# ChainSafe/lumenos

Hardware: AMD Instinct MI355X
Metric: prove_eval_seconds_16384x4096 (lower is better)
Workload: dtype u64; 1 GPU; Encode+Commit+InnerProduct(r,b)+QueryCols 16384x4096 LogN=14 L=12 K=2 rhoInv=2 queries=309; parallelism=1 GPU: the whole job resident in HBM

## Files before the change

lumenos_amd/csrc/lm_common.h:

```cpp
#pragma once
#include <hip/hip_runtime.h>

#include <algorithm>
#include <cstdarg>
#include <cstdint>
#include <cstdio>
#include <map>
#include <memory>
#include <mutex>
#include <set>
#include <string>
#include <utility>
#include <vector>

#include "../../include/lumenos_hip.h"
#include "lm_arith.h"
#include "lm_dev.h"

#define LM_MAX_LIMBS LUMEN_MAX_LIMBS

struct lm_modmap {
    uint32_t period;
    uint8_t idx[LM_MAX_LIMBS];
};

struct lm_mods {
    mod_t m[LM_MAX_LIMBS];
};

struct lm_prof_entry {
    double total_ms = 0;
    uint64_t launches = 0;
    uint64_t units = 0;
};

struct lm_galois_key {
    lm_dev<u64> d_key;
    lm_dev<uint32_t> d_index;
    lm_dev<uint32_t> d_inv_index;
};

struct lumen_set {
    uint32_t count = 0;
    uint32_t nl = 0;
    uint32_t logw = 0;
    u64 *d = nullptr;
    size_t words = 0;
    bool owner = true;
    lumen_ctx *home = nullptr;
};

struct lm_shared {
    std::recursive_mutex mu;
    lm_dev<tw_t> tw_fwd;
    lm_dev<tw_t> tw_inv;
    std::vector<uint64_t> roots;
    uint32_t fieldN = 0;
    lm_dev<tw_t> scal;
    std::map<uint64_t, lm_galois_key> gkeys;
    std::map<std::string, std::shared_ptr<void>> ext;
};

struct lm_tuning {
    uint32_t ks_batch = 64;
    uint32_t ks_lanes = 0;
    int32_t ks_fused_digits = -1;
    uint32_t ks_close_fused = 1;
    uint32_t debug = 0;
    uint32_t modup_tgroup = 3, moddown_tgroup = 1;
    uint32_t ks_placement = 6;
    uint32_t batch_chunks = 0;
    uint32_t rccl_shared_device = 0;
};

struct lumen_ctx {
    lm_tuning tune;
    std::recursive_mutex mu;
    std::shared_ptr<lm_shared> sh;
    int device = 0;
    hipStream_t stream = nullptr;
    hipStream_t stream2 = nullptr;
    hipEvent_t ev_fork = nullptr, ev_join = nullptr;
    hipStream_t stream_aux = nullptr;
    hipEvent_t ev_aux = nullptr;
    hipEvent_t ev_xdep = nullptr;
    uint32_t aux_digests = 0;
    const u64 *aux_lo = nullptr, *aux_hi = nullptr;
    uint8_t *aux_host = nullptr;
    size_t aux_host_cap = 0;
    void *stage_host = nullptr;
    size_t stage_cap = 0;
    hipEvent_t ev_stage = nullptr;
    void *io_host[2] = {nullptr, nullptr};
    hipEvent_t ev_io[2] = {nullptr, nullptr};
    uint32_t logN = 0, N = 0, L = 0, K = 0;
    uint64_t T = 0;
    uint64_t mod[LM_MAX_LIMBS] = {0};
    uint64_t psi[LM_MAX_LIMBS] = {0};
    lm_mods mods;
    tw_t ninv[LM_MAX_LIMBS];
    std::vector<uint64_t> &roots;
    uint32_t &fieldN;
    std::map<uint64_t, lm_galois_key> &gkeys;
    std::map<std::string, std::shared_ptr<void>> &ext;
    uint64_t mul_counter = 0;
    std::map<std::string, lm_dev<unsigned char>> scratch;
    struct pool_block {
        void *p;
        hipEvent_t ready;
    };
    std::multimap<size_t, pool_block> pool;
    size_t pool_bytes = 0;
    std::set<const void *> lds_attr_done;
    bool prof = false;
    std::map<std::string, lm_prof_entry> prof_tab;
    struct pending_ev {
        std::string name;
        hipEvent_t a, b;
        uint64_t units;
    };
    std::vector<pending_ev> prof_pending;
    std::vector<hipEvent_t> ev_pool;
    hipEvent_t tm0 = nullptr, tm1 = nullptr;
    std::string err;
    explicit lumen_ctx(std::shared_ptr<lm_shared> s)
        : sh(std::move(s)), roots(sh->roots), fieldN(sh->fieldN), gkeys(sh->gkeys), ext(sh->ext) {}
};

static inline size_t lm_ctw(const lumen_ctx *ctx, const lumen_set *s);
#define LM_FULL_WIDTH(ctx, set, what) \
    LM_CHECK(ctx, (set)->logw == 0, "%s: lane-sharded set (1/%u of every limb) where a full-width set is required", what, 1u << (set)->logw)

#define LM_ENTER(ctx)                                             \
    std::lock_guard<std::recursive_mutex> lm_lock_((ctx)->mu);    \
    (void)hipSetDevice((ctx)->device);                            \
    (void)hipGetLastError()
#define LM_SHARED_LOCK(ctx) std::lock_guard<std::recursive_mutex> lm_shlock_((ctx)->sh->mu)

template <class T>
static inline std::shared_ptr<T> lm_ext_get(lumen_ctx *ctx, const std::string &key) {
    LM_SHARED_LOCK(ctx);
    auto it = ctx->ext.find(key);
    return it == ctx->ext.end() ? std::shared_ptr<T>() : std::static_pointer_cast<T>(it->second);
}
static inline void lm_ext_put(lumen_ctx *ctx, const std::string &key, std::shared_ptr<void> v) {
    LM_SHARED_LOCK(ctx);
    ctx->ext[key] = std::move(v);
}

static inline size_t lm_ctw(const lumen_ctx *ctx, const lumen_set *s) { return (size_t)2 * s->nl * (ctx->N >> s->logw); }

void lm_sync_all(lumen_ctx *ctx);
void *lm_stage(lumen_ctx *ctx, size_t bytes);
int lm_h2d_staged(lumen_ctx *ctx, void *dev, const void *host, size_t bytes);
bool lm_host_is_pinned(const void *p);
int lm_h2d(lumen_ctx *ctx, void *dev, const void *host, size_t bytes);
int lm_d2h(lumen_ctx *ctx, void *host, const void *dev, size_t bytes, bool wait);
int lm_h2d_rows(lumen_ctx *ctx, void *dev, size_t dpitch, const void *host, size_t spitch, size_t width, size_t height);

int lm_fail(lumen_ctx *ctx, const char *fmt, ...);
extern thread_local std::string lm_global_err;

#define LM_HIP(ctx, call)                                                                  \
    do {                                                                                   \
        hipError_t e_ = (call);                                                            \
        if (e_ != hipSuccess)                                                              \
            return lm_fail(ctx, "%s failed: %s (%s:%d)", #call, hipGetErrorString(e_),     \
                           __FILE__, __LINE__);                                            \
    } while (0)

#define LM_CHECK(ctx, cond, ...)                    \
    do {                                            \
        if (!(cond)) return lm_fail(ctx, __VA_ARGS__); \
    } while (0)

template <class... P, class... A>
static inline int lm_launch_flat(lumen_ctx *ctx, void (*kernel)(P...), size_t threads, A &&...args) {
    hipLaunchKernelGGL(kernel, dim3((uint32_t)((threads + 255) / 256)), dim3(256), 0, ctx->stream, std::forward<A>(args)...);
    LM_HIP(ctx, hipGetLastError());
    return 0;
}

struct lm_set_guard {
    lumen_ctx *ctx;
    lumen_set *s;
    lm_set_guard(lumen_ctx *c, lumen_set *x) : ctx(c), s(x) {}
    ~lm_set_guard() {
        if (s) lumen_set_destroy(ctx, s);
    }
    lumen_set *release() {
        lumen_set *r = s;
        s = nullptr;
        return r;
    }
    lm_set_guard(lm_set_guard &&o) : ctx(o.ctx), s(o.release()) {}
    lm_set_guard &operator=(const lm_set_guard &) = delete;
};

void lm_set_release_async(lumen_ctx *ctx, lumen_set *set);

void *lm_scratch(lumen_ctx *ctx, const char *name, size_t bytes);
void lm_scratch_adopt(lumen_ctx *ctx, const char *name, void *p, size_t bytes);

struct lm_prof_scope {
    lumen_ctx *ctx;
    const char *name;
    uint64_t units;
    hipEvent_t a = nullptr;
    lm_prof_scope(lumen_ctx *c, const char *n, uint64_t u);
    ~lm_prof_scope();
};
void lm_prof_resolve(lumen_ctx *ctx);

static inline uint64_t h_mulmod(uint64_t a, uint64_t b, uint64_t q) {
    return (uint64_t)(((u128)a * b) % q);
}
static inline uint64_t h_powmod(uint64_t a, uint64_t e, uint64_t q) {
    uint64_t r = 1 % q;
    a %= q;
    while (e) {
        if (e & 1) r = h_mulmod(r, a, q);
        a = h_mulmod(a, a, q);
        e >>= 1;
    }
    return r;
}
static inline uint64_t h_invmod(uint64_t a, uint64_t q) { return h_powmod(a, q - 2, q); }
static inline tw_t h_tw(uint64_t w, uint64_t q) {
    tw_t t;
    t.w = w;
    t.wp = (u64)((((u128)w) << 64) / q);
    return t;
}
static inline uint64_t h_r64_mod(uint64_t q) { return (uint64_t)((((u128)1) << 64) % q); }
static inline uint64_t h_p_mod(const lumen_ctx *ctx, uint64_t q) {
    uint64_t P = 1 % q;
    for (uint32_t a = 0; a < ctx->K; a++) P = h_mulmod(P, ctx->mod[ctx->L + a] % q, q);
    return P;
}
static inline uint32_t h_bitrev(uint32_t x, int bits) {
    uint32_t r = 0;
    for (int i = 0; i < bits; i++) r = (r << 1) | ((x >> i) & 1);
    return r;
}

int lm_launch_ntt(lumen_ctx *ctx, u64 *d, uint32_t npoly, const lm_modmap &map, bool inverse);
struct lm_ninv_t;
int lm_launch_ntt_strided(lumen_ctx *ctx, const u64 *src, size_t src_poly_stride, u64 *dst,
                          size_t dst_poly_stride, uint32_t npoly, const lm_modmap &map, bool inverse,
                          const char *prof_name, const lm_ninv_t *inv_scale = nullptr);
int lm_launch_ntt_subring(lumen_ctx *ctx, uint32_t logn, const tw_t *tw, tw_t ninv_scale, const u64 *src,
                          size_t src_poly_stride, u64 *dst, size_t dst_poly_stride, uint32_t npoly,
                          uint32_t mod_idx, bool inverse, const mod_t *explicit_mod = nullptr);
mod_t lm_make_mod(uint64_t q);
void lm_build_tw(uint64_t q, uint64_t psi, uint32_t logN, std::vector<tw_t> &fwd, std::vector<tw_t> &inv);
int lm_rescale_polys(lumen_ctx *ctx, const u64 *src, uint32_t nl, u64 *dst, uint32_t target,
                     uint32_t npoly, u64 *work, u64 *tbuf);
int lm_rescale_coef_ready(lumen_ctx *ctx);
int lm_rescale_polys_from_coef(lumen_ctx *ctx, const u64 *coef, uint32_t nl, u64 *dst, uint32_t target, uint32_t npoly);
lm_modmap lm_map_q(uint32_t nl);
lm_modmap lm_map_p(const lumen_ctx *ctx);
int lm_encode_dev(lumen_ctx *ctx, const lumen_set *matrix, const u64 *dzero, uint32_t rho_inv, lumen_set **encoded);
int lm_poly_eval_check(lumen_ctx *ctx, const uint64_t *values, uint32_t rows, uint32_t count, uint64_t first_column,
                       uint32_t cols, const char *what);
int lm_poly_eval_enqueue(lumen_ctx *ctx, const uint64_t *values, uint32_t rows, uint32_t count, uint64_t first_column,
                         uint32_t cols, uint64_t z, const char *what);
int lm_poly_eval_finish(lumen_ctx *ctx, uint64_t *partial);
hipEvent_t lm_ev_get(lumen_ctx *ctx);
```

lumenos_amd/csrc/lm_ctx.hip:

```cpp
#include <cstring>
#include <thread>

#include "lm_ntt_plan.h"

thread_local std::string lm_global_err;

int lm_fail(lumen_ctx *ctx, const char *fmt, ...) {
    char buf[1024];
    va_list ap;
    va_start(ap, fmt);
    vsnprintf(buf, sizeof(buf), fmt, ap);
    va_end(ap);
    if (ctx) ctx->err = buf;
    lm_global_err = buf;
    fprintf(stderr, "[lumenos_hip] error: %s\n", buf);
    return 1;
}

void *lm_scratch(lumen_ctx *ctx, const char *name, size_t bytes) {
    auto &e = ctx->scratch[name];
    if (e && e.count() >= bytes) return e.get();
    if (e) lm_sync_all(ctx);
    return e.alloc(ctx, bytes, name) ? nullptr : e.get();
}

void lm_scratch_adopt(lumen_ctx *ctx, const char *name, void *p, size_t bytes) {
    auto &e = ctx->scratch[name];
    if (e.get() == p) (void)e.release();
    if (e) lm_sync_all(ctx);
    e = lm_dev<unsigned char>((unsigned char *)p, bytes);
}

void lm_sync_all(lumen_ctx *ctx) {
    if (ctx->stream) hipStreamSynchronize(ctx->stream);
    if (ctx->stream2) hipStreamSynchronize(ctx->stream2);
    if (ctx->stream_aux) hipStreamSynchronize(ctx->stream_aux);
}

void *lm_stage(lumen_ctx *ctx, size_t bytes) {
    if (ctx->ev_stage) hipEventSynchronize(ctx->ev_stage);
    if (ctx->stage_cap < bytes) {
        if (ctx->stage_host) hipHostFree(ctx->stage_host);
        ctx->stage_host = nullptr, ctx->stage_cap = 0;
        if (hipHostMalloc(&ctx->stage_host, bytes, hipHostMallocDefault) != hipSuccess) {
            lm_fail(ctx, "hipHostMalloc(%zu) for host staging failed", bytes);
            return nullptr;
        }
        ctx->stage_cap = bytes;
    }
    return ctx->stage_host;
}

int lm_h2d_staged(lumen_ctx *ctx, void *dev, const void *host, size_t bytes) {
    void *h = lm_stage(ctx, bytes);
    if (!h) return 1;
    memcpy(h, host, bytes);
    LM_HIP(ctx, hipMemcpyAsync(dev, h, bytes, hipMemcpyHostToDevice, ctx->stream));
    LM_HIP(ctx, hipEventRecord(ctx->ev_stage, ctx->stream));
    return 0;
}

hipEvent_t lm_ev_get(lumen_ctx *ctx) {
    if (!ctx->ev_pool.empty()) {
        hipEvent_t e = ctx->ev_pool.back();
        ctx->ev_pool.pop_back();
        return e;
    }
    hipEvent_t e = nullptr;
    hipEventCreate(&e);
    return e;
}

lm_prof_scope::lm_prof_scope(lumen_ctx *c, const char *n, uint64_t u) : ctx(c), name(n), units(u) {
    if (!ctx->prof) return;
    a = lm_ev_get(ctx);
    hipEventRecord(a, ctx->stream);
}
lm_prof_scope::~lm_prof_scope() {
    if (!ctx->prof || !a) return;
    hipEvent_t b = lm_ev_get(ctx);
    hipEventRecord(b, ctx->stream);
    ctx->prof_pending.push_back({name, a, b, units});
}

void lm_prof_resolve(lumen_ctx *ctx) {
    if (ctx->prof_pending.empty()) return;
    for (auto &p : ctx->prof_pending) {
        float ms = 0;
        if (hipEventSynchronize(p.b) == hipSuccess && hipEventElapsedTime(&ms, p.a, p.b) == hipSuccess) {
            auto &e = ctx->prof_tab[p.name];
            e.total_ms += ms;
            e.launches += 1;
            e.units += p.units;
        } else {
            (void)hipGetLastError();
        }
        ctx->ev_pool.push_back(p.a);
        ctx->ev_pool.push_back(p.b);
    }
    ctx->prof_pending.clear();
}

lm_modmap lm_map_q(uint32_t nl) {
    lm_modmap m;
    m.period = nl;
    for (uint32_t i = 0; i < LM_MAX_LIMBS; i++) m.idx[i] = (uint8_t)(i < nl ? i : 0);
    return m;
}

lm_modmap lm_map_p(const lumen_ctx *ctx) {
    lm_modmap m;
    m.period = ctx->K;
    for (uint32_t i = 0; i < LM_MAX_LIMBS; i++) m.idx[i] = (uint8_t)(ctx->L + (i < ctx->K ? i : 0));
    return m;
}

mod_t lm_make_mod(uint64_t q) {
    mod_t m;
    m.q = q;
    m.qinv64 = (u64)((((u128)1) << 64) / q);
    u64 inv = 1;
    for (int it = 0; it < 6; it++) inv *= 2 - (u64)q * inv;
    m.qneg = (u64)0 - inv;
    u64 r = h_r64_mod(q);
    m.r2 = h_mulmod(r, r, q);
    return m;
}

void lm_build_tw(uint64_t q, uint64_t psi, uint32_t logN, std::vector<tw_t> &fwd, std::vector<tw_t> &inv) {
    uint32_t N = 1u << logN;
    fwd.resize(N);
    inv.resize(N);
    uint64_t psi_inv = h_invmod(psi, q), cf = 1, cb = 1;
    for (uint32_t j = 0; j < N; j++) {
        uint32_t r = h_bitrev(j, (int)logN);
        fwd[r] = h_tw(cf, q);
        inv[r] = h_tw(cb, q);
        cf = h_mulmod(cf, psi, q);
        cb = h_mulmod(cb, psi_inv, q);
    }
}

static void pool_drain(lumen_ctx *ctx) {
    for (auto &kv : ctx->pool) {
        hipFree(kv.second.p);
        if (kv.second.ready) ctx->ev_pool.push_back(kv.second.ready);
    }
    ctx->pool.clear();
    ctx->pool_bytes = 0;
}

static int ctx_private_init(lumen_ctx *ctx) {
    LM_HIP(ctx, hipSetDevice(ctx->device));
    LM_HIP(ctx, hipStreamCreate(&ctx->stream));
    LM_HIP(ctx, hipStreamCreate(&ctx->stream2));
    LM_HIP(ctx, hipEventCreateWithFlags(&ctx->ev_fork, hipEventDisableTiming));
    LM_HIP(ctx, hipEventCreateWithFlags(&ctx->ev_join, hipEventDisableTiming));
    LM_HIP(ctx, hipStreamCreate(&ctx->stream_aux));
    LM_HIP(ctx, hipEventCreateWithFlags(&ctx->ev_aux, hipEventDisableTiming));
    LM_HIP(ctx, hipEventCreateWithFlags(&ctx->ev_stage, hipEventDisableTiming));
    LM_HIP(ctx, hipEventCreateWithFlags(&ctx->ev_xdep, hipEventDisableTiming));
    LM_HIP(ctx, hipEventCreate(&ctx->tm0));
    LM_HIP(ctx, hipEventCreate(&ctx->tm1));
    return 0;
}

static int tuning_set(lm_tuning &t, const char *name, long v) {
    const std::string n(name ? name : "");
    auto in = [&](long lo, long hi) { return v >= lo && v <= hi; };
    if (n == "LUMEN_KS_BATCH") {
        if (!in(1, 4096)) return 2;
        t.ks_batch = (uint32_t)v;
    } else if (n == "LUMEN_KS_LANES") {
        if (!in(0, 2)) return 2;
        t.ks_lanes = (uint32_t)v;
    } else if (n == "LUMEN_KS_FUSED_DIGITS") {
        if (v > LM_MAX_LIMBS) return 2;
        t.ks_fused_digits = v >= 0 ? (int32_t)v : -1;
    } else if (n == "LUMEN_KS_CLOSE_FUSED") {
        if (!in(0, 1)) return 2;
        t.ks_close_fused = (uint32_t)v;
    } else if (n == "LUMEN_DEBUG") {
        t.debug = v != 0;
    } else if (n == "LUMEN_MODUP_TGROUP") {
        if (!in(1, 31)) return 2;
        t.modup_tgroup = (uint32_t)v;
    } else if (n == "LUMEN_MODDOWN_TGROUP") {
        if (!in(1, 31)) return 2;
        t.moddown_tgroup = (uint32_t)v;
    } else if (n == "LUMEN_KS_PLACEMENT") {
        if (!in(0, 32)) return 2;
        t.ks_placement = (uint32_t)v;
    } else if (n == "LUMEN_BATCH_CHUNKS") {
        if (!in(0, 4096)) return 2;
        t.batch_chunks = (uint32_t)v;
    } else {
        return 1;
    }
    return 0;
}
static void tuning_from_env(lm_tuning &t) {
    for (const char *n : {"LUMEN_KS_BATCH", "LUMEN_KS_LANES", "LUMEN_KS_FUSED_DIGITS", "LUMEN_KS_CLOSE_FUSED", "LUMEN_DEBUG",
                          "LUMEN_MODUP_TGROUP", "LUMEN_MODDOWN_TGROUP", "LUMEN_KS_PLACEMENT", "LUMEN_BATCH_CHUNKS"}) {
        const char *e = getenv(n);
        if (e && *e && tuning_set(t, n, atol(e)))
            fprintf(stderr, "[lumenos_hip] %s=%s is out of range: ignored\n", n, e);
    }
}

extern "C" int lumen_ctx_set_tuning(lumen_ctx *ctx, const char *name, long value) {
    LM_CHECK(nullptr, ctx && name, "lumen_ctx_set_tuning: NULL argument");
    LM_ENTER(ctx);
    const int rc = tuning_set(ctx->tune, name, value);
    LM_CHECK(ctx, rc != 1, "unknown tuning switch %s", name);
    LM_CHECK(ctx, rc == 0, "tuning switch %s: value %ld is out of range (nothing changed)", name, value);
    return 0;
}

extern "C" int lumen_test_allow_shared_device_rccl(lumen_ctx *ctx, int on) {
    LM_CHECK(nullptr, ctx, "lumen_test_allow_shared_device_rccl: NULL ctx");
    LM_ENTER(ctx);
    ctx->tune.rccl_shared_device = on != 0;
    return 0;
}

extern "C" int lumen_ctx_wait(lumen_ctx *ctx, lumen_ctx *other) {
    LM_CHECK(nullptr, ctx && other, "lumen_ctx_wait: NULL argument");
    if (ctx == other) return 0;
    hipEvent_t ev;
    {
        LM_ENTER(other);
        LM_HIP(other, hipEventRecord(other->ev_xdep, other->stream));
        ev = other->ev_xdep;
    }
    LM_ENTER(ctx);
    LM_CHECK(ctx, ctx->device == other->device, "lumen_ctx_wait: contexts on devices %d and %d", ctx->device, other->device);
    LM_HIP(ctx, hipStreamWaitEvent(ctx->stream, ev, 0));
    return 0;
}

extern "C" int lumen_ctx_create(const lumen_params_desc *desc, lumen_ctx **out) {
    if (!desc || !out) return lm_fail(nullptr, "lumen_ctx_create: NULL argument");
    *out = nullptr;
    LM_CHECK(nullptr, desc->abi_version == LUMEN_ABI_VERSION, "ABI version mismatch: got %u want %u",
             desc->abi_version, LUMEN_ABI_VERSION);
    LM_CHECK(nullptr, lm_logn_supported(desc->log_n) || lm_logn_split_supported(desc->log_n),
             "log_n %u unsupported: kernels are instantiated for N = 2^8 and 2^10..2^14, and the server's path and the key "
             "switch for N = 2^15",
             desc->log_n);
    LM_CHECK(nullptr, desc->num_q >= 1 && desc->num_q + desc->num_p <= LM_MAX_LIMBS,
             "bad limb counts L=%u K=%u", desc->num_q, desc->num_p);
    int ndev = 0;
    if (hipGetDeviceCount(&ndev) != hipSuccess || ndev == 0)
        return lm_fail(nullptr, "no HIP device visible: the lumenos HIP path has no CPU fallback");
    LM_CHECK(nullptr, desc->device >= 0 && desc->device < ndev, "device %d out of range (have %d)",
             desc->device, ndev);
    std::unique_ptr<lumen_ctx, void (*)(lumen_ctx *)> guard(new lumen_ctx(std::make_shared<lm_shared>()),
                                                            lumen_ctx_destroy);
    lumen_ctx *ctx = guard.get();
    tuning_from_env(ctx->tune);
    ctx->device = desc->device;
    ctx->logN = desc->log_n;
    ctx->N = 1u << desc->log_n;
    ctx->L = desc->num_q;
    ctx->K = desc->num_p;
    ctx->T = desc->plaintext_modulus;
    uint32_t LK = ctx->L + ctx->K, N = ctx->N;
    uint64_t two_n = 2ull * N;
    for (uint32_t i = 0; i < LK; i++) {
        uint64_t q = desc->moduli[i], psi = desc->psi[i];
        const uint64_t qmax = UINT64_MAX / lm_q_bound_factor(desc->log_n);
        if (q < (1ull << 20) || q > qmax || (q & (two_n - 1)) != 1)
            return lm_fail(nullptr, "modulus %u (%llu) must be == 1 mod 2N and below %llu", i,
                           (unsigned long long)q, (unsigned long long)qmax);
        if (h_powmod(psi, N, q) != q - 1)
            return lm_fail(nullptr, "psi[%u] is not a primitive 2N-th root of unity", i);
        ctx->mod[i] = q;
        ctx->psi[i] = psi;
        ctx->mods.m[i] = lm_make_mod(q);
        ctx->ninv[i] = h_tw(h_invmod(N % q, q), q);
    }
    for (uint32_t i = LK; i < LM_MAX_LIMBS; i++) ctx->mods.m[i] = ctx->mods.m[0];
    if (int rc = ctx_private_init(ctx)) return rc;
    std::vector<tw_t> f, b, fwd, inv;
    for (uint32_t i = 0; i < LK; i++) {
        lm_build_tw(ctx->mod[i], ctx->psi[i], ctx->logN, f, b);
        fwd.insert(fwd.end(), f.begin(), f.end());
        inv.insert(inv.end(), b.begin(), b.end());
    }
    lm_layout_tw(fwd, ctx->logN);
    lm_layout_tw(inv, ctx->logN);
    if (ctx->sh->tw_fwd.upload(ctx, fwd, "the forward twiddles") || ctx->sh->tw_inv.upload(ctx, inv, "the inverse twiddles")) return 1;
    *out = guard.release();
    return 0;
}

extern "C" int lumen_ctx_clone(lumen_ctx *src, lumen_ctx **out) {
    if (!src || !out) return lm_fail(nullptr, "lumen_ctx_clone: NULL argument");
    *out = nullptr;
    LM_ENTER(src);
    std::unique_ptr<lumen_ctx, void (*)(lumen_ctx *)> guard(new lumen_ctx(src->sh), lumen_ctx_destroy);
    lumen_ctx *ctx = guard.get();
    ctx->tune = src->tune;
    ctx->device = src->device;
    ctx->logN = src->logN, ctx->N = src->N, ctx->L = src->L, ctx->K = src->K, ctx->T = src->T;
    memcpy(ctx->mod, src->mod, sizeof(ctx->mod));
    memcpy(ctx->psi, src->psi, sizeof(ctx->psi));
    ctx->mods = src->mods;
    memcpy(ctx->ninv, src->ninv, sizeof(ctx->ninv));
    if (int rc = ctx_private_init(ctx)) {
        src->err = ctx->err;
        return rc;
    }
    *out = guard.release();
    return 0;
}

extern "C" void lumen_ctx_destroy(lumen_ctx *ctx) {
    if (!ctx) return;
    {
        LM_ENTER(ctx);
        lm_sync_all(ctx);
        ctx->scratch.clear();
        pool_drain(ctx);
        lm_prof_resolve(ctx);
        for (hipEvent_t e : ctx->ev_pool) hipEventDestroy(e);
        if (ctx->tm0) hipEventDestroy(ctx->tm0);
        if (ctx->tm1) hipEventDestroy(ctx->tm1);
        if (ctx->aux_host) hipHostFree(ctx->aux_host);
        if (ctx->stage_host) hipHostFree(ctx->stage_host);
        for (int i = 0; i < 2; i++) {
            if (ctx->io_host[i]) hipHostFree(ctx->io_host[i]);
            if (ctx->ev_io[i]) hipEventDestroy(ctx->ev_io[i]);
        }
        if (ctx->ev_stage) hipEventDestroy(ctx->ev_stage);
        if (ctx->ev_xdep) hipEventDestroy(ctx->ev_xdep);
        if (ctx->ev_aux) hipEventDestroy(ctx->ev_aux);
        if (ctx->stream_aux) hipStreamDestroy(ctx->stream_aux);
        if (ctx->ev_fork) hipEventDestroy(ctx->ev_fork);
        if (ctx->ev_join) hipEventDestroy(ctx->ev_join);
        if (ctx->stream2) hipStreamDestroy(ctx->stream2);
        if (ctx->stream) hipStreamDestroy(ctx->stream);
        ctx->sh.reset();
    }
    delete ctx;
}

extern "C" int lumen_ctx_trim(lumen_ctx *ctx) {
    LM_CHECK(nullptr, ctx, "lumen_ctx_trim: NULL ctx");
    LM_ENTER(ctx);
    LM_CHECK(ctx, !ctx->aux_digests, "lumen_ctx_trim: a lumen_leaf_digests_begin job is in flight");
    lm_sync_all(ctx);
    for (auto it = ctx->scratch.begin(); it != ctx->scratch.end();) {
        if (it->first == "digests_async" || it->first == "group_digests") {
            ++it;
            continue;
        }
        it = ctx->scratch.erase(it);
    }
    pool_drain(ctx);
    return 0;
}

extern "C" int lumen_ctx_scratch_info(lumen_ctx *ctx, const char *name, void **ptr, size_t *bytes) {
    LM_CHECK(nullptr, ctx && name && ptr, "lumen_ctx_scratch_info: NULL argument");
    LM_ENTER(ctx);
    auto it = ctx->scratch.find(name);
    *ptr = it == ctx->scratch.end() ? nullptr : it->second.get();
    if (bytes) *bytes = it == ctx->scratch.end() ? 0 : it->second.count();
    return 0;
}

extern "C" const char *lumen_last_error(const lumen_ctx *ctx) {
    return ctx ? ctx->err.c_str() : lm_global_err.c_str();
}

extern "C" int lumen_sync(lumen_ctx *ctx) {
    LM_CHECK(nullptr, ctx, "lumen_sync: NULL ctx");
    LM_ENTER(ctx);
    LM_HIP(ctx, hipStreamSynchronize(ctx->stream));
    return 0;
}

extern "C" uint64_t lumen_mul_counter(const lumen_ctx *ctx) { return ctx ? ctx->mul_counter : 0; }

extern "C" int lumen_set_create(lumen_ctx *ctx, uint32_t count, uint32_t num_limbs, lumen_set **out) {
    return lumen_set_create_lanes(ctx, count, num_limbs, 0, out);
}

extern "C" int lumen_set_create_lanes(lumen_ctx *ctx, uint32_t count, uint32_t num_limbs, uint32_t log_world,
                                      lumen_set **out) {
    LM_CHECK(nullptr, ctx && out, "lumen_set_create: NULL argument");
    LM_ENTER(ctx);
    LM_CHECK(ctx, num_limbs >= 1 && num_limbs <= ctx->L, "num_limbs %u out of range [1,%u]", num_limbs, ctx->L);
    LM_CHECK(ctx, log_world <= 6 && (ctx->N >> log_world) >= 64, "a lane shard of 1/%u of N = %u is narrower than 64 coefficients",
             1u << log_world, ctx->N);
    lumen_set *s = new lumen_set();
    s->count = count;
    s->nl = num_limbs;
    s->logw = log_world;
    s->words = (size_t)count * 2 * num_limbs * (ctx->N >> log_world);
    s->home = ctx;
    if (s->words) {
        const size_t bytes = s->words * sizeof(u64);
        auto it = ctx->pool.find(bytes);
        if (it != ctx->pool.end()) {
            s->d = (u64 *)it->second.p;
            if (hipEvent_t ready = it->second.ready) {
                (void)hipStreamWaitEvent(ctx->stream, ready, 0);
                (void)hipStreamWaitEvent(ctx->stream2, ready, 0);
                (void)hipStreamWaitEvent(ctx->stream_aux, ready, 0);
                ctx->ev_pool.push_back(ready);
            }
            ctx->pool.erase(it);
            ctx->pool_bytes -= bytes;
        } else {
            hipError_t e = hipMalloc((void **)&s->d, bytes);
            if (e != hipSuccess && !ctx->pool.empty()) {
                (void)hipGetLastError();
                lm_sync_all(ctx);
                pool_drain(ctx);
                e = hipMalloc((void **)&s->d, bytes);
            }
            if (e != hipSuccess) {
                (void)hipGetLastError();
                delete s;
                return lm_fail(ctx, "hipMalloc(%zu bytes) for a %u x %u-limb set failed: %s", bytes, count,
                               num_limbs, hipGetErrorString(e));
            }
        }
    }
    *out = s;
    return 0;
}

extern "C" void lumen_set_destroy(lumen_ctx *ctx, lumen_set *set) {
    if (!set) return;
    if (ctx) {
        LM_ENTER(ctx);
        hipStreamSynchronize(ctx->stream);
        hipStreamSynchronize(ctx->stream2);
        if (ctx->aux_digests && set->d && set->d < ctx->aux_hi && set->d + set->words > ctx->aux_lo)
            hipStreamSynchronize(ctx->stream_aux);
        if (set->owner && set->d) {
            const size_t bytes = set->words * sizeof(u64);
            if (ctx == set->home && ctx->pool_bytes + bytes <= ((size_t)96 << 30)) {
                ctx->pool.emplace(bytes, lumen_ctx::pool_block{set->d, nullptr});
                ctx->pool_bytes += bytes;
            } else {
                hipFree(set->d);
            }
        }
    } else if (set->owner && set->d) {
        hipFree(set->d);
    }
    delete set;
}

void lm_set_release_async(lumen_ctx *ctx, lumen_set *set) {
    if (!set) return;
    LM_ENTER(ctx);
    const size_t bytes = set->words * sizeof(u64);
    const bool hashing = ctx->aux_digests && set->d && set->d < ctx->aux_hi && set->d + set->words > ctx->aux_lo;
    if (!set->owner || !set->d || ctx != set->home || hashing || ctx->pool_bytes + bytes > ((size_t)96 << 30)) {
        lumen_set_destroy(ctx, set);
        return;
    }
    hipEvent_t ready = lm_ev_get(ctx);
    bool ok = ready && hipEventRecord(ctx->ev_join, ctx->stream2) == hipSuccess &&
              hipStreamWaitEvent(ctx->stream, ctx->ev_join, 0) == hipSuccess && hipEventRecord(ready, ctx->stream) == hipSuccess;
    if (!ok) {
        (void)hipGetLastError();
        if (ready) ctx->ev_pool.push_back(ready);
        lumen_set_destroy(ctx, set);
        return;
    }
    ctx->pool.emplace(bytes, lumen_ctx::pool_block{set->d, ready});
    ctx->pool_bytes += bytes;
    delete set;
}

extern "C" int lumen_set_slice(lumen_ctx *ctx, const lumen_set *set, uint32_t first, uint32_t n,
                               lumen_set **view) {
    LM_CHECK(nullptr, ctx && set && view, "lumen_set_slice: NULL argument");
    LM_ENTER(ctx);
    LM_CHECK(ctx, (uint64_t)first + n <= set->count, "slice [%u,%u) exceeds set of %u", first, first + n, set->count);
    lumen_set *v = new lumen_set();
    const size_t ctw = lm_ctw(ctx, set);
    v->count = n;
    v->nl = set->nl;
    v->logw = set->logw;
    v->d = set->d + (size_t)first * ctw;
    v->words = (size_t)n * ctw;
    v->owner = false;
    *view = v;
    return 0;
}

extern "C" uint32_t lumen_set_count(const lumen_set *set) { return set ? set->count : 0; }
extern "C" uint32_t lumen_set_limbs(const lumen_set *set) { return set ? set->nl : 0; }
extern "C" uint32_t lumen_set_log_world(const lumen_set *set) { return set ? set->logw : 0; }
extern "C" void *lumen_set_device_ptr(const lumen_set *set) { return set ? set->d : nullptr; }

extern "C" void *lumen_host_alloc(size_t bytes) {
    void *p = nullptr;
    if (hipHostMalloc(&p, bytes ? bytes : 1, hipHostMallocDefault) != hipSuccess) {
        (void)hipGetLastError();
        lm_fail(nullptr, "hipHostMalloc(%zu) failed", bytes);
        return nullptr;
    }
    return p;
}
extern "C" void lumen_host_free(void *p) {
    if (p) hipHostFree(p);
}

static int host_limbs_move(uint64_t *flat, uint64_t *const *limbs, size_t n, size_t words, uint32_t threads, bool gather) {
    if (!n || !words) return 0;
    const size_t bytes = words * sizeof(uint64_t);
    size_t nthr = threads ? threads : std::max(1u, std::min(16u, std::thread::hardware_concurrency()));
    nthr = std::min(nthr, n);
    auto work = [=](size_t lo, size_t hi) {
        for (size_t i = lo; i < hi; i++) {
            if (gather) memcpy(flat + i * words, limbs[i], bytes);
            else memcpy(limbs[i], flat + i * words, bytes);
        }
    };
    if (nthr == 1) {
        work(0, n);
        return 0;
    }
    std::vector<std::thread> th;
    for (size_t t = 0; t < nthr; t++) th.emplace_back(work, n * t / nthr, n * (t + 1) / nthr);
    for (auto &x : th) x.join();
    return 0;
}
extern "C" int lumen_host_gather(uint64_t *dst, const uint64_t *const *limbs, size_t n, size_t words, uint32_t threads) {
    LM_CHECK(nullptr, (dst && limbs) || !n, "lumen_host_gather: NULL argument");
    for (size_t i = 0; i < n; i++) LM_CHECK(nullptr, limbs[i], "lumen_host_gather: limb %zu is NULL", i);
    return host_limbs_move(dst, const_cast<uint64_t *const *>(limbs), n, words, threads, true);
}
extern "C" int lumen_host_scatter(const uint64_t *src, uint64_t *const *limbs, size_t n, size_t words, uint32_t threads) {
    LM_CHECK(nullptr, (src && limbs) || !n, "lumen_host_scatter: NULL argument");
    for (size_t i = 0; i < n; i++) LM_CHECK(nullptr, limbs[i], "lumen_host_scatter: limb %zu is NULL", i);
    return host_limbs_move(const_cast<uint64_t *>(src), limbs, n, words, threads, false);
}

bool lm_host_is_pinned(const void *p) {
    hipPointerAttribute_t a;
    if (hipPointerGetAttributes(&a, p) != hipSuccess) {
        (void)hipGetLastError();
        return false;
    }
    return a.type == hipMemoryTypeHost;
}

#define LM_IO_CHUNK ((size_t)64 << 20)
static void par_memcpy(void *dst, const void *src, size_t bytes) {
    const size_t nthr = bytes >= ((size_t)8 << 20) ? 4 : 1;
    if (nthr == 1) {
        memcpy(dst, src, bytes);
        return;
    }
    std::thread th[4];
    const size_t part = (bytes / nthr + 63) & ~(size_t)63;
    for (size_t t = 0; t < nthr; t++) {
        const size_t lo = std::min(bytes, t * part), hi = std::min(bytes, lo + part);
        th[t] = std::thread([=] { memcpy((char *)dst + lo, (const char *)src + lo, hi - lo); });
    }
    for (size_t t = 0; t < nthr; t++) th[t].join();
}

static int io_buffers(lumen_ctx *ctx) {
    for (int i = 0; i < 2; i++) {
        if (!ctx->io_host[i]) LM_HIP(ctx, hipHostMalloc(&ctx->io_host[i], LM_IO_CHUNK, hipHostMallocDefault));
        if (!ctx->ev_io[i]) LM_HIP(ctx, hipEventCreateWithFlags(&ctx->ev_io[i], hipEventDisableTiming));
    }
    return 0;
}

int lm_h2d(lumen_ctx *ctx, void *dev, const void *host, size_t bytes) {
    char *dst = (char *)dev;
    if (bytes <= ((size_t)1 << 20) || lm_host_is_pinned(host)) {
        LM_HIP(ctx, hipMemcpyAsync(dst, host, bytes, hipMemcpyHostToDevice, ctx->stream));
    } else {
        if (int rc = io_buffers(ctx)) return rc;
        int i = 0;
        for (size_t off = 0; off < bytes; off += LM_IO_CHUNK, i ^= 1) {
            const size_t len = std::min(LM_IO_CHUNK, bytes - off);
            LM_HIP(ctx, hipEventSynchronize(ctx->ev_io[i]));
            par_memcpy(ctx->io_host[i], (const char *)host + off, len);
            LM_HIP(ctx, hipMemcpyAsync(dst + off, ctx->io_host[i], len, hipMemcpyHostToDevice, ctx->stream));
            LM_HIP(ctx, hipEventRecord(ctx->ev_io[i], ctx->stream));
        }
    }
    LM_HIP(ctx, hipStreamSynchronize(ctx->stream));
    return 0;
}

int lm_h2d_rows(lumen_ctx *ctx, void *dev, size_t dpitch, const void *host, size_t spitch, size_t width, size_t height) {
    char *dst = (char *)dev;
    const char *src = (const char *)host;
    if (!width || !height) return 0;
    if (width * height <= ((size_t)1 << 20) || lm_host_is_pinned(host)) {
        LM_HIP(ctx, hipMemcpy2DAsync(dst, dpitch, src, spitch, width, height, hipMemcpyHostToDevice, ctx->stream));
    } else {
        LM_CHECK(ctx, width <= LM_IO_CHUNK, "lm_h2d_rows: a row of %zu bytes exceeds the bounce buffer", width);
        if (int rc = io_buffers(ctx)) return rc;
        const size_t per = LM_IO_CHUNK / width;
        int i = 0;
        for (size_t r = 0; r < height; r += per, i ^= 1) {
            const size_t nr = std::min(per, height - r);
            LM_HIP(ctx, hipEventSynchronize(ctx->ev_io[i]));
            if (spitch == width)
                par_memcpy(ctx->io_host[i], src + r * spitch, nr * width);
            else
                for (size_t k = 0; k < nr; k++) memcpy((char *)ctx->io_host[i] + k * width, src + (r + k) * spitch, width);
            LM_HIP(ctx, hipMemcpy2DAsync(dst + r * dpitch, dpitch, ctx->io_host[i], width, width, nr, hipMemcpyHostToDevice,
                                         ctx->stream));
            LM_HIP(ctx, hipEventRecord(ctx->ev_io[i], ctx->stream));
        }
    }
    LM_HIP(ctx, hipStreamSynchronize(ctx->stream));
    return 0;
}

extern "C" int lumen_set_upload(lumen_ctx *ctx, lumen_set *set, uint32_t first, uint32_t n,
                                const uint64_t *host) {
    LM_CHECK(nullptr, ctx && set && host, "lumen_set_upload: NULL argument");
    LM_ENTER(ctx);
    LM_CHECK(ctx, (uint64_t)first + n <= set->count, "upload range [%u,%u) exceeds set of %u", first, first + n, set->count);
    const size_t ctw = lm_ctw(ctx, set), bytes = (size_t)n * ctw * sizeof(u64);
    return lm_h2d(ctx, set->d + (size_t)first * ctw, host, bytes);
}

int lm_d2h(lumen_ctx *ctx, void *host, const void *dev, size_t bytes, bool wait) {
    const char *src = (const char *)dev;
    if (bytes <= ((size_t)1 << 20) || lm_host_is_pinned(host)) {
        LM_HIP(ctx, hipMemcpyAsync(host, src, bytes, hipMemcpyDeviceToHost, ctx->stream));
        if (wait || !lm_host_is_pinned(host)) LM_HIP(ctx, hipStreamSynchronize(ctx->stream));
        return 0;
    }
    if (int rc = io_buffers(ctx)) return rc;
    const size_t nchunks = (bytes + LM_IO_CHUNK - 1) / LM_IO_CHUNK;
    auto issue = [&](size_t k) -> int {
        const size_t off = k * LM_IO_CHUNK, len = std::min(LM_IO_CHUNK, bytes - off);
        LM_HIP(ctx, hipMemcpyAsync(ctx->io_host[k & 1], src + off, len, hipMemcpyDeviceToHost, ctx->stream));
        LM_HIP(ctx, hipEventRecord(ctx->ev_io[k & 1], ctx->stream));
        return 0;
    };
    if (nchunks)
        if (int rc = issue(0)) return rc;
    for (size_t k = 0; k < nchunks; k++) {
        if (k + 1 < nchunks)
            if (int rc = issue(k + 1)) return rc;
        const size_t off = k * LM_IO_CHUNK, len = std::min(LM_IO_CHUNK, bytes - off);
        LM_HIP(ctx, hipEventSynchronize(ctx->ev_io[k & 1]));
        par_memcpy((char *)host + off, ctx->io_host[k & 1], len);
    }
    return 0;
}

extern "C" int lumen_set_download(lumen_ctx *ctx, const lumen_set *set, uint32_t first, uint32_t n,
                                  uint64_t *host) {
    LM_CHECK(nullptr, ctx && set && host, "lumen_set_download: NULL argument");
    LM_ENTER(ctx);
    LM_CHECK(ctx, (uint64_t)first + n <= set->count, "download range [%u,%u) exceeds set of %u", first, first + n, set->count);
    const size_t ctw = lm_ctw(ctx, set), bytes = (size_t)n * ctw * sizeof(u64);
    return lm_d2h(ctx, host, set->d + (size_t)first * ctw, bytes, true);
}

__global__ void k_fill_random(u64 *d, size_t words, uint32_t N, uint32_t nl, lm_mods mods, u64 seed) {
    size_t i = (size_t)blockIdx.x * blockDim.x + threadIdx.x;
    size_t stride = (size_t)gridDim.x * blockDim.x;
    for (; i < words; i += stride) {
        uint32_t limb = (uint32_t)((i / N) % nl);
        u64 z = seed + 0x9e3779b97f4a7c15ull * (u64)(i + 1);
        z = (z ^ (z >> 30)) * 0xbf58476d1ce4e5b9ull;
        z = (z ^ (z >> 27)) * 0x94d049bb133111ebull;
        z ^= z >> 31;
        d[i] = lm_reduce(z, mods.m[limb].q, mods.m[limb].qinv64);
    }
}

extern "C" int lumen_set_fill_random(lumen_ctx *ctx, lumen_set *set, uint64_t seed) {
    LM_CHECK(nullptr, ctx && set, "lumen_set_fill_random: NULL argument");
    LM_ENTER(ctx);
    if (!set->words) return 0;
    hipLaunchKernelGGL(k_fill_random, dim3(2048), dim3(256), 0, ctx->stream, set->d, set->words,
                       ctx->N >> set->logw, set->nl, ctx->mods, (u64)seed);
    LM_HIP(ctx, hipGetLastError());
    return 0;
}

extern "C" int lumen_timer_start(lumen_ctx *ctx) {
    LM_CHECK(nullptr, ctx, "NULL ctx");
    LM_ENTER(ctx);
    LM_HIP(ctx, hipEventRecord(ctx->tm0, ctx->stream));
    return 0;
}

extern "C" int lumen_timer_stop(lumen_ctx *ctx, float *elapsed_ms) {
    LM_CHECK(nullptr, ctx && elapsed_ms, "NULL argument");
    LM_ENTER(ctx);
    LM_HIP(ctx, hipEventRecord(ctx->tm1, ctx->stream));
    LM_HIP(ctx, hipEventSynchronize(ctx->tm1));
    LM_HIP(ctx, hipEventElapsedTime(elapsed_ms, ctx->tm0, ctx->tm1));
    return 0;
}

extern "C" int lumen_prof_enable(lumen_ctx *ctx, int on) {
    LM_CHECK(nullptr, ctx, "NULL ctx");
    LM_ENTER(ctx);
    if (!on) lm_prof_resolve(ctx);
    ctx->prof = on != 0;
    return 0;
}

extern "C" int lumen_prof_reset(lumen_ctx *ctx) {
    LM_CHECK(nullptr, ctx, "NULL ctx");
    LM_ENTER(ctx);
    lm_prof_resolve(ctx);
    ctx->prof_tab.clear();
    return 0;
}

extern "C" size_t lumen_prof_names(lumen_ctx *ctx, char *buf, size_t cap) {
    if (!ctx) return 0;
    LM_ENTER(ctx);
    lm_prof_resolve(ctx);
    std::string all;
    for (auto &kv : ctx->prof_tab) {
        if (!all.empty()) all += ",";
        all += kv.first;
    }
    if (buf && cap) {
        size_t n = std::min(cap - 1, all.size());
        memcpy(buf, all.data(), n);
        buf[n] = 0;
    }
    return all.size();
}

extern "C" int lumen_prof_read(lumen_ctx *ctx, const char *kernel, double *total_ms,
                               uint64_t *launches, uint64_t *units) {
    LM_CHECK(nullptr, ctx && kernel, "NULL argument");
    LM_ENTER(ctx);
    lm_prof_resolve(ctx);
    auto it = ctx->prof_tab.find(kernel);
    lm_prof_entry e;
    if (it != ctx->prof_tab.end()) e = it->second;
    if (total_ms) *total_ms = e.total_ms;
    if (launches) *launches = e.launches;
    if (units) *units = e.units;
    return 0;
}
```

lumenos_amd/csrc/lm_innersum.hip:

```cpp
#include <algorithm>

#include "lm_ks_host.h"

__global__ __launch_bounds__(256) void k_acc_canon(u64 *__restrict__ acc, size_t pairs, uint32_t logN, uint32_t L, lm_mods mods) {
    const size_t stride = (size_t)gridDim.x * blockDim.x;
    for (size_t g = (size_t)blockIdx.x * blockDim.x + threadIdx.x; g < pairs; g += stride) {
        const u64 q = mods.m[(uint32_t)((g >> (logN - 1)) % L)].q;
        ulonglong2 v = *reinterpret_cast<ulonglong2 *>(acc + 2 * g);
        v.x = lm_csub(v.x, q), v.y = lm_csub(v.y, q);
        *reinterpret_cast<ulonglong2 *>(acc + 2 * g) = v;
    }
}

__global__ __launch_bounds__(256) void k_lazy_gather(const u64 *__restrict__ u, const u64 *__restrict__ cur, u64 *__restrict__ lazy,
                                                     const uint32_t *__restrict__ index, uint32_t B, uint32_t L, uint32_t K,
                                                     uint32_t pshift, uint32_t logN, uint32_t first, lm_mods mods) {
    const uint32_t N = 1u << logN, nq = L * 2 * B;
    const size_t total = (size_t)2 * B * (L + K) * (N / 2), stride = (size_t)gridDim.x * blockDim.x;
    for (size_t g = (size_t)blockIdx.x * blockDim.x + threadIdx.x; g < total; g += stride) {
        const uint32_t j = (uint32_t)(g & (N / 2 - 1)) * 2, limb = (uint32_t)(g >> (logN - 1));
        const uint32_t t = limb < nq ? limb / (2 * B) : L + (limb - nq) % K;
        const uint32_t pw = limb < nq ? limb % (2 * B) : (limb - nq) / K;
        const bool with_c = t < L && (pw & 1) == (u ? 0u : 1u);
        if (!u && !with_c) continue;
        const u64 q = mods.m[ks_mod_at(t, L, pshift)].q;
        const size_t o = ((size_t)limb << logN) + j;
        uint2 p;
        p.x = j, p.y = j + 1;
        if (index) p = *reinterpret_cast<const uint2 *>(index + j);
        ulonglong2 v;
        v.x = v.y = 0;
        if (!first) v = *reinterpret_cast<const ulonglong2 *>(lazy + o);
        if (u) v.x += u[((size_t)limb << logN) + p.x], v.y += u[((size_t)limb << logN) + p.y];
        if (with_c) {
            const u64 *c = cur + (((size_t)pw * L + t) << logN);
            v.x += c[p.x], v.y += c[p.y];
        }
        v.x = lm_csub(lm_csub(v.x, 2 * q), q), v.y = lm_csub(lm_csub(v.y, 2 * q), q);
        *reinterpret_cast<ulonglong2 *>(lazy + o) = v;
    }
}

namespace {

int acc_canon(lumen_ctx *ctx, u64 *acc, size_t words, uint32_t L) {
    if (!words) return 0;
    hipLaunchKernelGGL(k_acc_canon, dim3(2048), dim3(256), 0, ctx->stream, acc, words / 2, ctx->logN, L, ctx->mods);
    LM_HIP(ctx, hipGetLastError());
    return 0;
}


bool is_plain(const lumen_ctx *ctx, uint32_t batch, uint32_t n) { return batch == 1 && n && !(n & (n - 1)) && n <= ctx->N; }

template <class Fn>
int sum_walk(const lumen_ctx *ctx, uint32_t batch, uint32_t n, Fn &&fn) {
    if (is_plain(ctx, batch, n)) {
        uint64_t gal[64];
        const uint32_t cnt = lumen_inner_sum_galois_elements(ctx, n, gal);
        for (uint32_t r = 0; r < cnt; r++)
            if (int rc = fn((uint64_t)0, gal[r])) return rc;
        return 0;
    }
    for (uint32_t i = 0, j = n; j > 1; i++, j >>= 1) {
        const uint64_t term = (j & 1) ? lumen_galois_element(ctx, (int64_t)((uint64_t)(n - (n & ((2u << i) - 1))) * batch)) : 0;
        if (int rc = fn(term, lumen_galois_element(ctx, (int64_t)((uint64_t)batch << i)))) return rc;
    }
    return 0;
}

struct SumPlan {
    struct Step {
        const lm_galois_key *dbl = nullptr, *term = nullptr;
    } it[32];
    uint32_t cnt = 0;
    uint64_t last_el = 0;
    bool lazy = false;
};

int sum_plan(lumen_ctx *ctx, uint32_t batch, uint32_t n, SumPlan *p) {
    return sum_walk(ctx, batch, n, [&](uint64_t term, uint64_t dbl) {
        SumPlan::Step &st = p->it[p->cnt++];
        if (term) {
            if (int rc = ks_find_key(ctx, term, &st.term)) return rc;
            p->lazy = true;
        }
        p->last_el = dbl;
        return ks_find_key(ctx, dbl, &st.dbl);
    });
}

int general_check(lumen_ctx *ctx, uint32_t batch, uint32_t n, const char *what) {
    LM_CHECK(ctx, batch >= 1 && n >= 1, "%s: batch size %u and length %u must both be at least 1", what, batch, n);
    LM_CHECK(ctx, ctx->K >= 1, "parameters have no special primes: key switching unavailable");
    LM_CHECK(ctx, ctx->K <= 2, "key switching supports 1 or 2 special primes (have %u)", ctx->K);
    if (is_plain(ctx, batch, n)) return 0;
    LM_CHECK(ctx, (uint64_t)batch * n <= ctx->N / 2, "%s: batch size %u x length %u spans beyond the slot row of %u slots", what, batch, n,
             ctx->N / 2);
    return 0;
}


int lazy_blocks(lumen_ctx *ctx, const KsRun &run, u64 **lazy) {
    const size_t bytes = (size_t)run.Bmax * 2 * (ctx->L + ctx->K) * ctx->N * 8;
    lazy[0] = (u64 *)lm_scratch(ctx, "ks_lazy", bytes);
    lazy[1] = run.lanes > 1 ? (u64 *)lm_scratch(ctx, "ks_lazy_b", bytes) : lazy[0];
    return lazy[0] && lazy[1] ? 0 : 1;
}

int lazy_gather(lumen_ctx *ctx, const u64 *u, const u64 *cur, u64 *lazy, const uint32_t *index, bool first, uint32_t B, KsTables *tb) {
    lm_prof_scope ps(ctx, "ks_lazy_gather", (uint64_t)B);
    hipLaunchKernelGGL(k_lazy_gather, dim3(2048), dim3(256), 0, ctx->stream, u, cur, lazy, index, B, tb->nl, ctx->K, ctx->L - tb->nl,
                       ctx->logN, first ? 1u : 0u, ctx->mods);
    LM_HIP(ctx, hipGetLastError());
    return 0;
}

int identity_tables(lumen_ctx *ctx, std::shared_ptr<lm_galois_key> *out) {
    static const char *const NAME = "ks_identity";
    LM_SHARED_LOCK(ctx);
    auto gk = lm_ext_get<lm_galois_key>(ctx, NAME);
    if (!gk) {
        gk = std::make_shared<lm_galois_key>();
        std::vector<uint32_t> index(ctx->N);
        for (uint32_t i = 0; i < ctx->N; i++) index[i] = i;
        if (gk->d_index.upload(ctx, index, "the identity's index table") || gk->d_inv_index.upload(ctx, index, "the identity's index table"))
            return 1;
        lm_ext_put(ctx, NAME, gk);
    }
    *out = std::move(gk);
    return 0;
}

int lazy_close(lumen_ctx *ctx, const u64 *cur, u64 *out, u64 *lazy, uint32_t B, KsTables *tb, const KsScratch &s) {
    std::shared_ptr<lm_galois_key> id;
    if (int rc = identity_tables(ctx, &id)) return rc;
    if (int rc = lazy_gather(ctx, nullptr, cur, lazy, nullptr, false, B, tb)) return rc;
    if (int rc = rotate_p_to_coef(ctx, lazy, B, tb)) return rc;
    KsScratch sl = s;
    sl.u = lazy;
    return rotate_store(ctx, cur, out, B, *id, tb, sl);
}

int inner_sum_batch(lumen_ctx *ctx, u64 *acc, uint32_t B, const SumPlan &plan, KsTables *tb, const KsScratch &s, u64 *lazy,
                    u64 *close_out) {
    LM_CHECK(ctx, !close_out || (plan.cnt && !plan.lazy), "InnerSum has no rotation to close");
    u64 *cur = acc, *other = s.acc2;
    bool first = true;
    for (uint32_t r = 0; r < plan.cnt; r++) {
        const SumPlan::Step &st = plan.it[r];
        if (int rc = rotate_decompose(ctx, cur, B, tb, s)) return rc;
        if (st.term) {
            if (int rc = rotate_mac(ctx, cur, B, *st.term, tb, s)) return rc;
            if (int rc = lazy_gather(ctx, s.u, cur, lazy, st.term->d_index.get(), first, B, tb)) return rc;
            first = false;
        }
        if (close_out && r + 1 == plan.cnt)
            return rotate_close(ctx, cur, close_out, B, *st.dbl, plan.last_el, tb, s);
        if (int rc = rotate_add(ctx, cur, other, B, *st.dbl, tb, s)) return rc;
        std::swap(cur, other);
    }
    if (plan.lazy) {
        if (int rc = lazy_close(ctx, cur, other, lazy, B, tb, s)) return rc;
        std::swap(cur, other);
    }
    if (cur != acc)
        LM_HIP(ctx, hipMemcpyAsync(acc, cur, (size_t)B * 2 * tb->nl * ctx->N * 8, hipMemcpyDeviceToDevice, ctx->stream));
    return 0;
}

int check_inner_sum_level(lumen_ctx *ctx, const lumen_set *in, const char *what) {
    LM_FULL_WIDTH(ctx, in, what);
    LM_CHECK(ctx, in->nl == ctx->L, "%s is implemented at the top level only (set has %u of %u limbs)", what,
             in->nl, ctx->L);
    return 0;
}

int inner_sum_run(lumen_ctx *ctx, const lumen_set *in, uint32_t batch, uint32_t n, const char *general, lumen_set **out) {
    if (general) {
        if (int rc = general_check(ctx, batch, n, general)) return rc;
    } else {
        LM_CHECK(ctx, is_plain(ctx, batch, n), "InnerSum length %u is not a power of two <= N", n);
    }
    KsRun run;
    if (int rc = ks_run_open(ctx, in->count, in->nl, is_plain(ctx, batch, n) ? 1 : 2, false, &run)) return rc;
    SumPlan plan;
    if (in->count)
        if (int rc = sum_plan(ctx, batch, n, &plan)) return rc;
    lumen_set *o = nullptr;
    if (int rc = lumen_set_create(ctx, in->count, in->nl, &o)) return rc;
    lm_set_guard og(ctx, o);
    if (in->words)
        LM_HIP(ctx, hipMemcpyAsync(o->d, in->d, in->words * 8, hipMemcpyDeviceToDevice, ctx->stream));
    if (int rc = ks_run_scratch(ctx, &run)) return rc;
    u64 *lazy[2] = {nullptr, nullptr};
    if (plan.lazy)
        if (int rc = lazy_blocks(ctx, run, lazy)) return rc;
    const size_t ctw = (size_t)2 * in->nl * ctx->N;
    auto batch_fn = [&](uint32_t, uint32_t first, uint32_t B, const KsScratch &s, u64 *) {
        return inner_sum_batch(ctx, o->d + (size_t)first * ctw, B, plan, run.tb, s, lazy[&s == &run.s[1]], nullptr);
    };
    if (int rc = ks_run(ctx, run, in->count, ctw, batch_fn)) return rc;
    if (!plan.lazy)
        if (int rc = acc_canon(ctx, o->d, o->words, in->nl)) return rc;
    *out = og.release();
    return 0;
}

int matrix_inner_sum_run(lumen_ctx *ctx, const lumen_set *matrix, const uint64_t *pt, uint32_t rows, const char *general,
                         lumen_set **out) {
    if (general) {
        if (int rc = general_check(ctx, 1, rows, general)) return rc;
    } else {
        LM_CHECK(ctx, is_plain(ctx, 1, rows), "rows=%u is not a power of two <= N", rows);
    }
    KsRun run;
    if (int rc = ks_run_open(ctx, matrix->count, matrix->nl, 2, true, &run)) return rc;
    SumPlan plan;
    if (matrix->count)
        if (int rc = sum_plan(ctx, 1, rows, &plan)) return rc;
    u64 *ptT = nullptr;
    if (int rc = upload_ptT(ctx, pt, matrix->nl, &ptT)) return rc;
    const uint32_t N = ctx->N, L = matrix->nl, target = std::min<uint32_t>(2, L);
    lumen_set *o = nullptr;
    if (int rc = lumen_set_create(ctx, matrix->count, target, &o)) return rc;
    lm_set_guard og(ctx, o);
    const size_t ctw = (size_t)2 * L * N, octw = (size_t)2 * target * N;
    if (int rc = ks_run_scratch(ctx, &run)) return rc;
    u64 *lazy[2] = {nullptr, nullptr};
    if (plan.lazy)
        if (int rc = lazy_blocks(ctx, run, lazy)) return rc;
    u64 *work = (u64 *)lm_scratch(ctx, "rescale_work", run.group_bytes);
    u64 *tbuf = (u64 *)lm_scratch(ctx, "rescale_t", (size_t)run.group * 2 * N * 8);
    if (!work || !tbuf) return 1;
    bool close = false;
    if (L > target && rows > 1 && ctx->tune.ks_close_fused && !plan.lazy && !lm_is_split(ctx->logN)) {
        const int rc = lm_rescale_coef_ready(ctx);
        if (rc && rc != 2) return rc;
        close = rc == 0;
    }
    auto batch_fn = [&](uint32_t g0, uint32_t first, uint32_t B, const KsScratch &s, u64 *a) {
        if (int rc = launch_mul_plain(ctx, matrix->d + (size_t)(g0 + first) * ctw, a, ptT, (size_t)B * ctw, L, B))
            return rc;
        return inner_sum_batch(ctx, a, B, plan, run.tb, s, lazy[&s == &run.s[1]], close ? work + (size_t)first * ctw : nullptr);
    };
    auto end_of_group = [&](uint32_t g0, uint32_t gn) {
        if (close)
            return lm_rescale_polys_from_coef(ctx, work, L, o->d + (size_t)g0 * octw, target, gn * 2);
        if (L > target) return lm_rescale_polys(ctx, run.acc, L, o->d + (size_t)g0 * octw, target, gn * 2, work, tbuf);
        if (!plan.lazy)
            if (int rc = acc_canon(ctx, run.acc, (size_t)gn * ctw, L)) return rc;
        LM_HIP(ctx, hipMemcpyAsync(o->d + (size_t)g0 * octw, run.acc, (size_t)gn * ctw * 8, hipMemcpyDeviceToDevice, ctx->stream));
        return 0;
    };
    if (int rc = ks_run(ctx, run, matrix->count, ctw, batch_fn, end_of_group)) return rc;
    *out = og.release();
    return 0;
}

}

extern "C" int lumen_inner_sum_general(lumen_ctx *ctx, const lumen_set *in, uint32_t batch_size, uint32_t n, lumen_set **out) {
    LM_CHECK(nullptr, ctx && in && out, "lumen_inner_sum_general: NULL argument");
    LM_ENTER(ctx);
    if (int rc = check_level_of_chain(ctx, in, "InnerSum")) return rc;
    return inner_sum_run(ctx, in, batch_size, n, "lumen_inner_sum_general", out);
}

extern "C" int lumen_matrix_inner_sum_general(lumen_ctx *ctx, const lumen_set *matrix, const uint64_t *pt, uint32_t rows,
                                              lumen_set **out) {
    LM_CHECK(nullptr, ctx && matrix && pt && out, "lumen_matrix_inner_sum_general: NULL argument");
    LM_ENTER(ctx);
    if (int rc = check_level_of_chain(ctx, matrix, "matrixInnerSumEval")) return rc;
    return matrix_inner_sum_run(ctx, matrix, pt, rows, "lumen_matrix_inner_sum_general", out);
}

extern "C" uint32_t lumen_inner_sum_general_elements(const lumen_ctx *ctx, uint32_t batch_size, uint32_t n, uint64_t *gal_els) {
    if (!ctx || !gal_els) return 0;
    if (!is_plain(ctx, batch_size, n) && (!batch_size || !n || (uint64_t)batch_size * n > ctx->N / 2)) return 0;
    uint32_t cnt = 0;
    sum_walk(ctx, batch_size, n, [&](uint64_t term, uint64_t dbl) {
        for (uint64_t g : {term, dbl})
            if (g > 1 && std::find(gal_els, gal_els + cnt, g) == gal_els + cnt) gal_els[cnt++] = g;
        return 0;
    });
    return cnt;
}

extern "C" int lumen_inner_sum(lumen_ctx *ctx, const lumen_set *in, uint32_t n, lumen_set **out) {
    LM_CHECK(nullptr, ctx && in && out, "lumen_inner_sum: NULL argument");
    LM_ENTER(ctx);
    if (int rc = check_inner_sum_level(ctx, in, "InnerSum")) return rc;
    return inner_sum_run(ctx, in, 1, n, nullptr, out);
}

extern "C" int lumen_inner_sum_at_level(lumen_ctx *ctx, const lumen_set *in, uint32_t n, lumen_set **out) {
    LM_CHECK(nullptr, ctx && in && out, "lumen_inner_sum_at_level: NULL argument");
    LM_ENTER(ctx);
    if (int rc = check_level_of_chain(ctx, in, "InnerSum")) return rc;
    return inner_sum_run(ctx, in, 1, n, nullptr, out);
}

extern "C" int lumen_matrix_inner_sum(lumen_ctx *ctx, const lumen_set *matrix, const uint64_t *pt,
                                      uint32_t rows, lumen_set **out) {
    LM_CHECK(nullptr, ctx && matrix && pt && out, "lumen_matrix_inner_sum: NULL argument");
    LM_ENTER(ctx);
    if (int rc = check_inner_sum_level(ctx, matrix, "matrixInnerSumEval")) return rc;
    return matrix_inner_sum_run(ctx, matrix, pt, rows, nullptr, out);
}

extern "C" int lumen_matrix_inner_sum_at_level(lumen_ctx *ctx, const lumen_set *matrix, const uint64_t *pt,
                                               uint32_t rows, lumen_set **out) {
    LM_CHECK(nullptr, ctx && matrix && pt && out, "lumen_matrix_inner_sum_at_level: NULL argument");
    LM_ENTER(ctx);
    if (int rc = check_level_of_chain(ctx, matrix, "matrixInnerSumEval")) return rc;
    return matrix_inner_sum_run(ctx, matrix, pt, rows, nullptr, out);
}
```

lumenos_amd/csrc/lm_keyswitch.hip:

```cpp
#include <cstdlib>
#include <cstring>

#include "lm_ks_host.h"

__device__ __forceinline__ u32 bx_v(u128 A, u128 M, u64 y0, u64 y1, u64 m0, u64 m1) {
    const u128 D1 = A >= M ? A - M : M - A, D2 = 2 * M - A;
    if ((u64)(D1 >> 64) >= 8 && (u64)(D2 >> 64) >= 8) return A >= M ? 1u : 0u;
    double vf = 0.0;
    vf += (double)y0 / (double)m0;
    vf += (double)y1 / (double)m1;
    return (u32)(u64)vf;
}

__device__ __forceinline__ void pack_pair(u64 a, u64 b, u64 m0, u64 m1, u128 M, u64 &hi, u64 &lo) {
    u64 l1, h1, l2, h2;
    mul128(a, m1, l1, h1);
    mul128(b, m0, l2, h2);
    const u128 A = (((u128)h1 << 64) | l1) + (((u128)h2 << 64) | l2);
    const u32 v = bx_v(A, M, a, b, m0, m1);
    const u128 W = A + (v == 0 ? 2 * M : (v == 1 ? M : (u128)0));
    hi = (u64)(W >> LM_W_SPLIT), lo = (u64)W & ((1ull << LM_W_SPLIT) - 1);
}

__global__ __launch_bounds__(256) void k_pack_v(u64 *__restrict__ y, size_t poly_stride, uint32_t npoly,
                                                uint32_t ngroups, uint32_t group_limbs, uint32_t first_mod,
                                                uint32_t nlimbs_total, uint32_t logN, lm_mods mods) {
    const uint32_t N = 1u << logN;
    const size_t total = (size_t)npoly * ngroups * (N / 2), stride = (size_t)gridDim.x * blockDim.x;
    for (size_t g = (size_t)blockIdx.x * blockDim.x + threadIdx.x; g < total; g += stride) {
        const uint32_t i = (uint32_t)(g & (N / 2 - 1)) * 2;
        const uint32_t grp = (uint32_t)((g >> (logN - 1)) % ngroups), p = (uint32_t)((g >> (logN - 1)) / ngroups);
        const uint32_t l0 = grp * group_limbs;
        if (l0 + 1 >= nlimbs_total) continue;
        u64 *y0 = y + (size_t)p * poly_stride + (size_t)l0 * N + i;
        const ulonglong2 av = *reinterpret_cast<const ulonglong2 *>(y0);
        const ulonglong2 bv = *reinterpret_cast<const ulonglong2 *>(y0 + N);
        const u64 m0 = mods.m[first_mod + l0].q, m1 = mods.m[first_mod + l0 + 1].q;
        u64 Ml, Mh;
        mul128(m0, m1, Ml, Mh);
        const u128 M = ((u128)Mh << 64) | Ml;
        ulonglong2 hv, lv;
#pragma unroll
        for (int e = 0; e < 2; e++) {
            const u64 a = e ? av.y : av.x, b = e ? bv.y : bv.x;
            u64 hi, lo;
            pack_pair(a, b, m0, m1, M, hi, lo);
            if (e) hv.y = hi, lv.y = lo;
            else hv.x = hi, lv.x = lo;
        }
        *reinterpret_cast<ulonglong2 *>(y0) = hv;
        *reinterpret_cast<ulonglong2 *>(y0 + N) = lv;
    }
}

template <int LOGN>
__global__ LM_GEOM_BOUNDS(lm_geom_lds(LOGN)) void k_intt_pack(const u64 *__restrict__ acc, u64 *coef, uint32_t B,
                                                                  uint32_t L, uint32_t nf, lm_mods mods,
                                                                  lm_ninv_t yscale, const tw_t *__restrict__ tw_all) {
    extern __shared__ __attribute__((aligned(16))) u64 sm[];
    constexpr uint32_t N = 1u << LOGN;
    const uint32_t tid = threadIdx.x;
    if (blockIdx.x >= B * nf) {
        const uint32_t k = blockIdx.x - B * nf, l = 2 * nf + k / B, b = k % B;
        const u64 *p = acc + (((size_t)b * 2 + 1) * L + l) * N;
        u64 *o = coef + ((size_t)b * L + l) * N;
        const lm_qc q = lm_make_qc(mods.m[l]);
        const tw_t sc = yscale.t[l];
        auto ld = [&](uint32_t i0, u64 *v, int count) { lm_load_run(p, i0, v, count); };
        auto st = [&](uint32_t i, u64 v) { o[i] = lm_shoup_cs(v, sc, q.q, q.nq); };
        lm_ntt_inverse<LOGN>(sm, tw_all + (size_t)l * N, q, tid, ld, st);
        return;
    }
    const uint32_t d = blockIdx.x / B, b = blockIdx.x % B;
    const uint32_t l0 = 2 * d, l1 = l0 + 1;
    const u64 *c1 = acc + ((size_t)b * 2 + 1) * L * N;
    u64 *o0 = coef + ((size_t)b * L + l0) * N;
    const lm_qc q0 = lm_make_qc(mods.m[l0]);
    const tw_t s0 = yscale.t[l0];
    {
        const u64 *p = c1 + (size_t)l0 * N;
        auto ld = [&](uint32_t i0, u64 *v, int count) { lm_load_run(p, i0, v, count); };
        auto st = [&](uint32_t i, u64 v) { o0[i] = lm_shoup_cs(v, s0, q0.q, q0.nq); };
        lm_ntt_inverse<LOGN>(sm, tw_all + (size_t)l0 * N, q0, tid, ld, st);
    }
    __syncthreads();
    {
        const lm_qc q1 = lm_make_qc(mods.m[l1]);
        const tw_t s1 = yscale.t[l1];
        const u64 *p = c1 + (size_t)l1 * N;
        u64 Ml, Mh;
        mul128(q0.q, q1.q, Ml, Mh);
        auto uni = [](u64 x) {
            return (u64)(uint32_t)__builtin_amdgcn_readfirstlane((int)(uint32_t)x) |
                   (u64)(uint32_t)__builtin_amdgcn_readfirstlane((int)(uint32_t)(x >> 32)) << 32;
        };
        const u128 M = ((u128)uni(Mh) << 64) | uni(Ml);
        auto ld = [&](uint32_t i0, u64 *v, int count) { lm_load_run(p, i0, v, count); };
        constexpr int R_LAST = lm_pass_r(LOGN, 0), LOG_T0 = LOGN - R_LAST;
        constexpr int PF = (1 << R_LAST) * 5 / 8;
        struct pack_t {
            u64 *o0;
            const lm_qc &q0, &q1;
            tw_t s1;
            u128 M;
            u64 y0[PF];
            __device__ __forceinline__ void pre(uint32_t w) {
#pragma unroll
                for (int k = 0; k < PF; k++) y0[k] = o0[w + ((uint32_t)k << LOG_T0)];
            }
            __device__ __forceinline__ void operator()(uint32_t i, u64 v, int k) {
                const u64 y1 = lm_shoup_cs(v, s1, q1.q, q1.nq);
                uint32_t j = i;
                asm volatile("" : "+v"(j));
                const u64 a = k < PF ? y0[k < PF ? k : 0] : o0[j];
                u64 hi, lo;
                pack_pair(a, y1, q0.q, q1.q, M, hi, lo);
                o0[j] = hi, o0[j + N] = lo;
                if (k >= PF && (k & 1)) asm volatile("" ::: "memory");
            }
        } st{o0, q0, q1, s1, M, {}};
        uint32_t tid1 = tid;
        asm volatile("" : "+v"(tid1));
        lm_ntt_inverse<LOGN>(sm, tw_all + (size_t)l1 * N, q1, tid1, ld, st);
    }
}

template <int LOGN>
__global__ LM_GEOM_BOUNDS(lm_geom_fwd(LOGN)) void k_modup_ntt(const u64 *__restrict__ coef, const u64 *__restrict__ acc,
                                                    u64 *__restrict__ ext, const bx_t *__restrict__ bx,
                                                    uint32_t B, uint32_t L, uint32_t K, uint32_t beta, uint32_t pshift,
                                                    const uint32_t *__restrict__ work, lm_mods mods,
                                                    const tw_t *__restrict__ tw_all) {
    extern __shared__ __attribute__((aligned(16))) u64 sm[];
    constexpr uint32_t N = 1u << LOGN;
    const uint32_t tid = threadIdx.x, LK = L + K;
    const lm_half<LOGN> hf = lm_half_of_block<LOGN>();
    const uint32_t wk = work[hf.block];
    const uint32_t b = wk & 0xFFFF, d = (wk >> 16) & 0xFF, t = wk >> 24;
    const uint32_t mt = ks_mod_at(t, L, pshift);
    const bx_t c = bx[d * LK + t];
    u64 *o = ext + ks_ext_at(b, d, t, B, beta) * N + hf.off;
    const lm_qc qc = lm_make_qc(mods.m[mt]);
    const u64 *s0 = coef + ((size_t)b * L + d * K) * N;
    const u64 *s1 = c.ns == 2 ? s0 + N : s0;
    auto ld = [&](uint32_t i) { return bx_apply(c, s0[i], s1[i], qc); };
    auto out = [&](uint32_t j, u64 v0, u64 v1) {
        ulonglong2 y;
        y.x = v0, y.y = v1;
        *reinterpret_cast<ulonglong2 *>(o + j) = y;
    };
    if constexpr (LOGN == 14) {
        lm_w14_runs st{sm};
        auto after = [&](uint32_t i0, uint32_t) { lm_w14_linear_out(sm, tid, i0, out); };
        lm_ntt_forward_w14(sm, tw_all + (size_t)mt * N, qc, tid, ld, st, after);
    } else {
        lm_lds_runs st{sm};
        auto after = [&](uint32_t, uint32_t) { lm_linear_out<lm_tlog(LOGN)>(sm, tid, out); };
        lm_ntt_forward_half<LOGN>(sm, tw_all + (size_t)mt * N, qc, tid, hf, ld, st, after);
    }
}

#ifndef LM_MAC_COLS
#define LM_MAC_COLS 4
#endif
#ifndef LM_MAC_VEC
#define LM_MAC_VEC 1
#endif
#ifndef LM_MAC_PREFETCH
#define LM_MAC_PREFETCH 1
#endif
template <int VEC>
struct mac_vec;
template <>
struct mac_vec<1> {
    u64 v[1];
    static __device__ __forceinline__ mac_vec load(const u64 *p) { return mac_vec{{*p}}; }
    static __device__ __forceinline__ mac_vec load_once(const u64 *p) { return mac_vec{{__builtin_nontemporal_load(p)}}; }
    __device__ __forceinline__ void store(u64 *p) const { *p = v[0]; }
};
template <>
struct mac_vec<2> {
    u64 v[2];
    static __device__ __forceinline__ mac_vec load(const u64 *p) {
        const ulonglong2 a = *reinterpret_cast<const ulonglong2 *>(p);
        return mac_vec{{a.x, a.y}};
    }
    static __device__ __forceinline__ mac_vec load_once(const u64 *p) {
        return mac_vec{{__builtin_nontemporal_load(p), __builtin_nontemporal_load(p + 1)}};
    }
    __device__ __forceinline__ void store(u64 *p) const {
        ulonglong2 a;
        a.x = v[0], a.y = v[1];
        *reinterpret_cast<ulonglong2 *>(p) = a;
    }
};
struct mac_acc {
    u64 a0, a1, a3;
    u32 c0, c1;
    __device__ __forceinline__ void clear() { a0 = a1 = a3 = 0, c0 = c1 = 0; }
    __device__ __forceinline__ void value(u64 &lo, u64 &hi) const {
        lo = a0 + (a1 << 32);
        hi = a3 + c0 + (a1 >> 32) + ((u64)c1 << 32) + (lo < a0 ? 1 : 0);
    }
};
__device__ __forceinline__ void mac2(mac_acc &p, mac_acc &q, u64 x, u64 k0, u64 k1) {
    const u32 x0 = (u32)x, x1 = (u32)(x >> 32);
#if LM_ASM_SHOUP
    asm("v_mad_u64_u32 %[pa0], s[98:99], %[x0], %[k00], %[pa0]\n\t"
        "v_mad_u64_u32 %[qa0], s[90:91], %[x0], %[k10], %[qa0]\n\t"
        "v_mad_u64_u32 %[pa1], s[94:95], %[x0], %[k01], %[pa1]\n\t"
        "v_addc_co_u32_e64 %[pc0], s[96:97], %[pc0], 0, s[98:99]\n\t"
        "v_mad_u64_u32 %[qa1], s[92:93], %[x0], %[k11], %[qa1]\n\t"
        "v_addc_co_u32_e64 %[qc0], s[96:97], %[qc0], 0, s[90:91]\n\t"
        "v_mad_u64_u32 %[pa3], s[96:97], %[x1], %[k01], %[pa3]\n\t"
        "v_addc_co_u32_e64 %[pc1], s[96:97], %[pc1], 0, s[94:95]\n\t"
        "v_mad_u64_u32 %[pa1], s[98:99], %[x1], %[k00], %[pa1]\n\t"
        "v_addc_co_u32_e64 %[qc1], s[96:97], %[qc1], 0, s[92:93]\n\t"
        "v_mad_u64_u32 %[qa1], s[90:91], %[x1], %[k10], %[qa1]\n\t"
        "v_mad_u64_u32 %[qa3], s[96:97], %[x1], %[k11], %[qa3]\n\t"
        "v_addc_co_u32_e64 %[pc1], s[96:97], %[pc1], 0, s[98:99]\n\t"
        "v_addc_co_u32_e64 %[qc1], s[96:97], %[qc1], 0, s[90:91]"
        : [pa0] "+v"(p.a0), [pa1] "+v"(p.a1), [pa3] "+v"(p.a3), [pc0] "+v"(p.c0), [pc1] "+v"(p.c1),
          [qa0] "+v"(q.a0), [qa1] "+v"(q.a1), [qa3] "+v"(q.a3), [qc0] "+v"(q.c0), [qc1] "+v"(q.c1)
        : [x0] "v"(x0), [x1] "v"(x1), [k00] "v"((u32)k0), [k01] "v"((u32)(k0 >> 32)), [k10] "v"((u32)k1),
          [k11] "v"((u32)(k1 >> 32))
        : "s92", "s93", "s94", "s95", "s96", "s97", "s98", "s99", "s90", "s91");
#else
    auto one = [&](mac_acc &r, u64 k) {
        const u32 k0w = (u32)k, k1w = (u32)(k >> 32);
        u64 t = r.a0 + (u64)x0 * k0w;
        r.c0 += t < r.a0, r.a0 = t;
        t = r.a1 + (u64)x0 * k1w;
        r.c1 += t < r.a1, r.a1 = t;
        t = r.a1 + (u64)x1 * k0w;
        r.c1 += t < r.a1, r.a1 = t;
        r.a3 += (u64)x1 * k1w;
    };
    one(p, k0);
    one(q, k1);
#endif
}

__global__ __launch_bounds__(256) void k_ks_mac(const u64 *__restrict__ ext, const u64 *__restrict__ acc,
                                                const u64 *__restrict__ key, u64 *__restrict__ u, uint32_t B,
                                                uint32_t L, uint32_t K, uint32_t beta, uint32_t pshift,
                                                uint32_t key_beta, uint32_t logN, lm_mods mods) {
    typedef mac_vec<LM_MAC_VEC> vec;
    const uint32_t N = 1u << logN, LK = L + K;
    const uint32_t G = (B + LM_MAC_COLS - 1) / LM_MAC_COLS, per_limb = N / (256 * LM_MAC_VEC) ? N / (256 * LM_MAC_VEC) : 1;
    const uint32_t slices = per_limb * LK;
    uint32_t slice, z;
    if (slices % 8 == 0) {
        const uint32_t xcd = blockIdx.x & 7, j = blockIdx.x >> 3;
        z = j % G;
        slice = (j / G) * 8 + xcd;
    } else {
        z = blockIdx.x % G;
        slice = blockIdx.x / G;
    }
    const uint32_t i = ((slice % per_limb) * 256 + threadIdx.x) * LM_MAC_VEC;
    const uint32_t t = LK - 1 - slice / per_limb;
    const uint32_t mt = ks_mod_at(t, L, pshift);
    const uint32_t b0 = z * LM_MAC_COLS;
    if (i >= N) return;
    const mod_t md = mods.m[mt];
    const uint32_t own = t < L ? t / K : 0xFFFFFFFFu;
    mac_acc a0[LM_MAC_COLS][LM_MAC_VEC], a1[LM_MAC_COLS][LM_MAC_VEC];
#pragma unroll
    for (int c = 0; c < LM_MAC_COLS; c++)
#pragma unroll
        for (int e = 0; e < LM_MAC_VEC; e++) a0[c][e].clear(), a1[c][e].clear();
    struct digit_t {
        vec k0, k1, x[LM_MAC_COLS];
    };
    auto fetch = [&](uint32_t d) {
        digit_t g;
        g.k0 = vec::load(key + ks_key_at(d, 0, mt, key_beta) * N + i);
        g.k1 = vec::load(key + ks_key_at(d, 1, mt, key_beta) * N + i);
#pragma unroll
        for (int c = 0; c < LM_MAC_COLS; c++) {
            const uint32_t bc = b0 + c < B ? b0 + c : B - 1;
            g.x[c] = d == own ? vec::load(acc + ((size_t)(bc * 2 + 1) * L + t) * N + i)
                              : vec::load_once(ext + ks_ext_at(bc, d, t, B, beta) * N + i);
        }
        return g;
    };
    constexpr int PF = LM_MAC_PREFETCH;
    digit_t q[PF + 1];
#pragma unroll
    for (int j = 0; j < PF; j++)
        if ((uint32_t)j < beta) q[j] = fetch(j);
    for (uint32_t d0 = 0; d0 < beta; d0 += PF + 1) {
#pragma unroll
        for (int j = 0; j <= PF; j++) {
            const uint32_t d = d0 + j;
            if (d < beta) {
                if (d + PF < beta) q[(j + PF) % (PF + 1)] = fetch(d + PF);
#pragma unroll
                for (int c = 0; c < LM_MAC_COLS; c++)
#pragma unroll
                    for (int e = 0; e < LM_MAC_VEC; e++) mac2(a0[c][e], a1[c][e], q[j].x[c].v[e], q[j].k0.v[e], q[j].k1.v[e]);
            }
        }
    }
#pragma unroll
    for (int c = 0; c < LM_MAC_COLS; c++) {
        if (b0 + c < B) {
            u64 *o = u + ks_u_at((b0 + c) * 2, t, B, L, K) * N + i, *o1 = u + ks_u_at((b0 + c) * 2 + 1, t, B, L, K) * N + i;
            vec r0, r1;
#pragma unroll
            for (int e = 0; e < LM_MAC_VEC; e++) {
                u64 lo, hi;
                a0[c][e].value(lo, hi);
                r0.v[e] = lm_mont_reduce_wide(lo, hi, md.q, md.qneg, md.qinv64, beta);
                a1[c][e].value(lo, hi);
                r1.v[e] = lm_mont_reduce_wide(lo, hi, md.q, md.qneg, md.qinv64, beta);
            }
            r0.store(o);
            r1.store(o1);
        }
    }
}

template <int LOGN, bool ACCUMULATE>
__device__ __forceinline__ void moddown_body(const u64 *__restrict__ u, const u64 *__restrict__ acc_in,
                                             u64 *__restrict__ acc_out, const bx_t *__restrict__ bxp,
                                             const tw_t *__restrict__ pinv,
                                             const uint32_t *__restrict__ index,
                                             const uint32_t *__restrict__ inv_index,
                                             const uint32_t *__restrict__ work, uint32_t B,
                                             uint32_t L, uint32_t K, const lm_mods &mods,
                                             const tw_t *__restrict__ tw_all) {
    extern __shared__ __attribute__((aligned(16))) u64 sm[];
    constexpr uint32_t N = 1u << LOGN;
    const uint32_t tid = threadIdx.x;
    const lm_half<LOGN> hf = lm_half_of_block<LOGN>();
    const uint32_t wk = work[hf.block];
    const uint32_t pw = wk & 0xFFFF;
    const uint32_t t = wk >> 16;
    const uint32_t w = pw & 1;
    const bx_t c = bxp[t];
    const lm_qc qc = lm_make_qc(mods.m[t]);
    const u64 *up0 = u + ks_u_at(pw, L, B, L, K) * N;
    const u64 *up1 = c.ns == 2 ? up0 + N : up0;
    const u64 *uq = u + ks_u_at(pw, t, B, L, K) * N;
    const u64 *ain = acc_in + ((size_t)pw * L + t) * N;
    u64 *aout = acc_out + ((size_t)pw * L + t) * N;
    tw_t pi = pinv[t];
    pi.w = qc.q - pi.w, pi.wp = ~pi.wp;
    auto ld = [&](uint32_t i) { return bx_apply(c, up0[i], up1[i], qc); };
    if constexpr (LOGN == 14) {
        const uint32_t wave = tid >> 6, lane = tid & 63;
        const uint32_t jb0 = (uint32_t)__builtin_amdgcn_readfirstlane((int)(inv_index[(2 * wave) << 10] >> 10));
        const uint32_t jb1 = (uint32_t)__builtin_amdgcn_readfirstlane((int)(inv_index[(2 * wave + 1) << 10] >> 10));
        lm_w14_runs st{sm};
        auto after = [&](uint32_t i0h, uint32_t) {
            const uint32_t pb = LM_PAD((wave << 10) | (2 * lane));
            constexpr uint32_t CH = 4;
            const uint32_t i = (wave << 11) | i0h | (2 * lane);
            const uint32_t jb = i0h ? jb1 : jb0, sbase = wave << 10;
#pragma unroll
            for (uint32_t k0 = 0; k0 < 8; k0 += CH) {
                ulonglong2 uv[CH], cv[CH];
#pragma unroll
                for (uint32_t k = 0; k < CH; k++) {
                    uv[k] = *reinterpret_cast<const ulonglong2 *>(uq + i + 128 * (k0 + k));
                    if (w == 0) cv[k] = *reinterpret_cast<const ulonglong2 *>(ain + i + 128 * (k0 + k));
                }
#pragma unroll
                for (uint32_t k = 0; k < CH; k++) {
                    const uint32_t p = lm_w14_at(pb, 128 * (k0 + k));
                    const u64 a0 = w == 0 ? uv[k].x + cv[k].x : uv[k].x, a1 = w == 0 ? uv[k].y + cv[k].y : uv[k].y;
                    sm[p] = lm_shoup3<true>(sm[p], pi.w, pi.wp, qc.nq, a0);
                    sm[p + 1] = lm_shoup3<true>(sm[p + 1], pi.w, pi.wp, qc.nq, a1);
                }
                LM_W14_FENCE();
            }
            lm_wave_sync();
            uint2 p[8];
            ulonglong2 x[8];
#pragma unroll
            for (uint32_t k = 0; k < 8; k++) {
                const uint32_t j = (jb << 10) + 2 * lane + k * 128;
                p[k] = *reinterpret_cast<const uint2 *>(index + j);
                if constexpr (ACCUMULATE) x[k] = *reinterpret_cast<const ulonglong2 *>(ain + j);
            }
#pragma unroll
            for (uint32_t k = 0; k < 8; k++) {
                const uint32_t j = (jb << 10) + 2 * lane + k * 128;
                ulonglong2 y;
                if constexpr (ACCUMULATE) {
                    y.x = lm_csub(lm_csub(x[k].x + sm[LM_PAD(sbase | (p[k].x & 1023u))], 4 * qc.q), 2 * qc.q);
                    y.y = lm_csub(lm_csub(x[k].y + sm[LM_PAD(sbase | (p[k].y & 1023u))], 4 * qc.q), 2 * qc.q);
                } else {
                    y.x = lm_csub(lm_csub(lm_csub(sm[LM_PAD(sbase | (p[k].x & 1023u))], 4 * qc.q), 2 * qc.q), qc.q);
                    y.y = lm_csub(lm_csub(lm_csub(sm[LM_PAD(sbase | (p[k].y & 1023u))], 4 * qc.q), 2 * qc.q), qc.q);
                }
                *reinterpret_cast<ulonglong2 *>(aout + j) = y;
            }
        };
        lm_ntt_forward_w14(sm, tw_all + (size_t)t * N, qc, tid, ld, st, after);
    } else {
        constexpr int TLOG = lm_tlog(LOGN);
        constexpr int RUN = lm_fwd_run<TLOG>();
        static_assert(RUN <= 8, "lm_load_run moves at most 8 coefficients");
        struct storer_t {
            const u64 *uq, *ain;
            u64 *sm;
            const lm_qc &qc;
            tw_t pi;
            uint32_t w;
            u64 uv[RUN], cv[RUN];
            __device__ __forceinline__ void pre(uint32_t i0) {
                lm_load_run(uq, i0, uv, RUN);
                if (w == 0) lm_load_run(ain, i0, cv, RUN);
            }
            __device__ __forceinline__ void operator()(uint32_t i0, const u64 *v, int count) {
#pragma unroll
                for (int k = 0; k < RUN; k++)
                    if (k < count) {
                        const u64 add = w == 0 ? uv[k] + cv[k] : uv[k];
                        sm[LM_PAD(i0 + k)] = lm_shoup3<true>(v[k], pi.w, pi.wp, qc.nq, add);
                    }
            }
        } st{uq + hf.off, ain + hf.off, sm, qc, pi, w, {}, {}};
        constexpr uint32_t NW = lm_nthreads(TLOG) / 64, BLK = (1u << TLOG) / NW, IT = BLK / 128;
        const uint32_t wave = tid >> 6, lane = tid & 63;
        const uint32_t jb = NW > 1 ? (uint32_t)__builtin_amdgcn_readfirstlane((int)(inv_index[hf.off + wave * BLK] / BLK)) : 0u;
        auto after = [&](uint32_t, uint32_t) {
            uint2 p[IT];
            ulonglong2 x[IT];
#pragma unroll
            for (uint32_t k = 0; k < IT; k++) {
                const uint32_t j = jb * BLK + 2 * lane + k * 128;
                p[k] = *reinterpret_cast<const uint2 *>(index + j);
                if constexpr (ACCUMULATE) x[k] = *reinterpret_cast<const ulonglong2 *>(ain + j);
            }
            lm_wave_sync();
#pragma unroll
            for (uint32_t k = 0; k < IT; k++) {
                const uint32_t j = jb * BLK + 2 * lane + k * 128;
                ulonglong2 y;
                if constexpr (ACCUMULATE) {
                    y.x = lm_csub(lm_csub(x[k].x + sm[LM_PAD(lm_half_local<LOGN>(p[k].x))], 4 * qc.q), 2 * qc.q);
                    y.y = lm_csub(lm_csub(x[k].y + sm[LM_PAD(lm_half_local<LOGN>(p[k].y))], 4 * qc.q), 2 * qc.q);
                } else {
                    y.x = lm_csub(lm_csub(lm_csub(sm[LM_PAD(lm_half_local<LOGN>(p[k].x))], 4 * qc.q), 2 * qc.q), qc.q);
                    y.y = lm_csub(lm_csub(lm_csub(sm[LM_PAD(lm_half_local<LOGN>(p[k].y))], 4 * qc.q), 2 * qc.q), qc.q);
                }
                *reinterpret_cast<ulonglong2 *>(aout + j) = y;
            }
        };
        lm_ntt_forward_half<LOGN>(sm, tw_all + (size_t)t * N, qc, tid, hf, ld, st, after);
    }
}

#define LM_MODDOWN_PARAMS                                                                                                      \
    const u64 *__restrict__ u, const u64 *__restrict__ acc_in, u64 *__restrict__ acc_out, const bx_t *__restrict__ bxp,        \
        const tw_t *__restrict__ pinv, const uint32_t *__restrict__ index, const uint32_t *__restrict__ inv_index,             \
        const uint32_t *__restrict__ work, uint32_t B, uint32_t L, uint32_t K, lm_mods mods, const tw_t *__restrict__ tw_all
template <int LOGN>
__global__ LM_GEOM_BOUNDS(lm_geom_fwd(LOGN)) void k_moddown_ntt(LM_MODDOWN_PARAMS) {
    moddown_body<LOGN, true>(u, acc_in, acc_out, bxp, pinv, index, inv_index, work, B, L, K, mods, tw_all);
}
template <int LOGN>
__global__ LM_GEOM_BOUNDS(lm_geom_fwd(LOGN)) void k_rotdown_ntt(LM_MODDOWN_PARAMS) {
    moddown_body<LOGN, false>(u, acc_in, acc_out, bxp, pinv, index, inv_index, work, B, L, K, mods, tw_all);
}

namespace {

bx_t make_bx(const uint64_t *src, uint32_t ns, uint64_t t) {
    bx_t c;
    memset(&c, 0, sizeof(c));
    c.ns = ns;
    uint64_t m_mod_t = 1;
    for (uint32_t a = 0; a < ns; a++) m_mod_t = h_mulmod(m_mod_t, src[a] % t, t);
    c.b57 = h_tw((1ull << LM_W_SPLIT) % t, t);
    c.c_t = (t - h_mulmod(2 % t, m_mod_t, t)) % t;
    return c;
}

uint64_t hat_inv(const uint64_t *src, uint32_t ns, uint32_t a) {
    uint64_t h = 1;
    for (uint32_t b = 0; b < ns; b++)
        if (b != a) h = h_mulmod(h, src[b] % src[a], src[a]);
    return h_invmod(h, src[a]);
}

}

int get_tables(lumen_ctx *ctx, KsTables **out) { return get_tables_at(ctx, ctx->L, out); }

int get_tables_at(lumen_ctx *ctx, uint32_t nl, KsTables **out) {
    LM_SHARED_LOCK(ctx);
    LM_CHECK(ctx, nl >= 1 && nl <= ctx->L, "key switch at %u limbs: the chain has %u", nl, ctx->L);
    const std::string name = nl == ctx->L ? std::string("ks_tables") : "ks_tables:" + std::to_string(nl);
    auto it = ctx->ext.find(name);
    if (it != ctx->ext.end()) {
        *out = static_cast<KsTables *>(it->second.get());
        return 0;
    }
    const uint32_t L = nl, K = ctx->K, LK = L + K, pshift = ctx->L - nl, ctxLK = ctx->L + K;
    LM_CHECK(ctx, K >= 1 && K <= 2, "key switching supports 1 or 2 special primes (have %u)", K);
    auto sp = std::make_shared<KsTables>();
    KsTables &tb = *sp;
    tb.nl = L;
    tb.beta = (L + K - 1) / K;
    std::vector<bx_t> bx((size_t)tb.beta * LK);
    for (uint32_t d = 0; d < tb.beta; d++) {
        const uint32_t lo = d * K, hi = std::min(lo + K, L), ns = hi - lo;
        for (uint32_t t = 0; t < LK; t++) {
            bx_t c = make_bx(ctx->mod + lo, ns, ctx->mod[ks_mod_at(t, L, pshift)]);
            c.own = (t >= lo && t < hi) ? 1 : 0;
            bx[(size_t)d * LK + t] = c;
        }
    }
    for (uint32_t i = 0; i < LM_MAX_LIMBS; i++) tb.yscale.t[i] = ctx->ninv[i < ctxLK ? i : 0];
    for (uint32_t d = 0; d < tb.beta; d++) {
        const uint32_t lo = d * K, hi = std::min(lo + K, L), ns = hi - lo;
        for (uint32_t a = 0; a < ns; a++) {
            const uint64_t m = ctx->mod[lo + a];
            tb.yscale.t[lo + a] = h_tw(h_mulmod(ctx->ninv[lo + a].w, hat_inv(ctx->mod + lo, ns, a), m), m);
        }
    }
    for (uint32_t a = 0; a < K; a++) {
        const uint64_t m = ctx->mod[ctx->L + a];
        tb.yscale.t[ctx->L + a] = h_tw(h_mulmod(ctx->ninv[ctx->L + a].w, hat_inv(ctx->mod + ctx->L, K, a), m), m);
    }
    std::vector<bx_t> bxp(L);
    std::vector<tw_t> pinv(L);
    for (uint32_t t = 0; t < L; t++) {
        bxp[t] = make_bx(ctx->mod + ctx->L, K, ctx->mod[t]);
        const uint64_t q = ctx->mod[t];
        pinv[t] = h_tw(h_invmod(h_p_mod(ctx, q), q), q);
    }
    std::vector<uint16_t> pairs;
    for (uint32_t t = 0; t < LK; t++)
        for (uint32_t d = 0; d < tb.beta; d++)
            if (!bx[(size_t)d * LK + t].own) pairs.push_back((uint16_t)(d | (t << 8)));
    tb.pairs = pairs;
    if (tb.d_bx.upload(ctx, bx, "the key switch's extension constants") || tb.d_bxp.upload(ctx, bxp, "the key switch's lift constants") ||
        tb.d_pinv.upload(ctx, pinv, "the key switch's P^-1 table"))
        return 1;
    ctx->ext[name] = sp;
    *out = sp.get();
    return 0;
}

int lm_ks_tables_view(lumen_ctx *ctx, lm_ks_view *out) {
    KsTables *tb = nullptr;
    if (int rc = get_tables(ctx, &tb)) return rc;
    out->d_bxp = tb->d_bxp.get();
    out->d_pinv = tb->d_pinv.get();
    out->yscale = &tb->yscale;
    return 0;
}

int lm_launch_pack_v(lumen_ctx *ctx, u64 *y, size_t poly_stride, uint32_t npoly, uint32_t ngroups,
                     uint32_t group_limbs, uint32_t first_mod, uint32_t nlimbs_total) {
    hipLaunchKernelGGL(k_pack_v, dim3(2048), dim3(256), 0, ctx->stream, y, poly_stride, npoly, ngroups, group_limbs,
                       first_mod, nlimbs_total, ctx->logN, ctx->mods);
    LM_HIP(ctx, hipGetLastError());
    return 0;
}

namespace {

static int interleave_work_lists(lumen_ctx *ctx, const std::vector<std::vector<uint32_t>> &lists, size_t expect,
                                 const char *what, std::map<uint32_t, lm_dev<uint32_t>> &cache, uint32_t cache_key,
                                 const uint32_t **out) {
    std::vector<uint32_t> order;
    order.reserve(expect);
    std::vector<size_t> pos(8, 0);
    for (bool any = true; any;) {
        any = false;
        for (uint32_t x = 0; x < 8; x++)
            if (pos[x] < lists[x].size()) {
                order.push_back(lists[x][pos[x]++]);
                any = true;
            }
    }
    LM_CHECK(ctx, order.size() == expect, "%s work list is inconsistent", what);
    lm_dev<uint32_t> d;
    if (int rc = d.upload(ctx, order, "a key-switch work list")) return rc;
    *out = (cache[cache_key] = std::move(d)).get();
    return 0;
}

static int modup_work_list(lumen_ctx *ctx, KsTables *tb, uint32_t B, const uint32_t **out) {
    const uint32_t LM_MODUP_TGROUP = ctx->tune.modup_tgroup;
    LM_SHARED_LOCK(ctx);
    LM_CHECK(ctx, B >= 1 && B <= 65535 && tb->beta <= 255 && tb->nl + ctx->K <= 255,
             "key-switch batch of %u columns (beta %u) does not fit the packed work list", B, tb->beta);
    const uint32_t cache_key = B | (LM_MODUP_TGROUP << 16);
    auto it = tb->d_work.find(cache_key);
    if (it != tb->d_work.end()) {
        *out = it->second.get();
        return 0;
    }
    const uint32_t LK = tb->nl + ctx->K, beta = tb->beta;
    std::vector<std::vector<uint8_t>> need(beta);
    for (uint16_t pr : tb->pairs) need[pr & 0xFF].push_back((uint8_t)(pr >> 8));
    std::vector<std::vector<uint32_t>> lists(8);
    for (uint32_t x = 0; x < 8; x++)
        for (uint32_t t0 = 0; t0 < LK; t0 += LM_MODUP_TGROUP)
            for (uint32_t b = x; b < B; b += 8)
                for (uint32_t d = 0; d < beta; d++)
                    for (uint8_t t : need[d])
                        if (t >= t0 && t < t0 + LM_MODUP_TGROUP) lists[x].push_back(b | (d << 16) | ((uint32_t)t << 24));
    return interleave_work_lists(ctx, lists, (size_t)B * tb->pairs.size(), "extension", tb->d_work, cache_key, out);
}

static int moddown_work_list(lumen_ctx *ctx, KsTables *tb, uint32_t B, const uint32_t **out) {
    const uint32_t LM_MODDOWN_TGROUP = ctx->tune.moddown_tgroup;
    LM_SHARED_LOCK(ctx);
    LM_CHECK(ctx, B >= 1 && 2 * (uint64_t)B <= 65535, "key-switch batch of %u columns does not fit the packed work list", B);
    const uint32_t cache_key = B | (LM_MODDOWN_TGROUP << 17);
    auto it = tb->d_work_down.find(cache_key);
    if (it != tb->d_work_down.end()) {
        *out = it->second.get();
        return 0;
    }
    const uint32_t L = tb->nl;
    std::vector<std::vector<uint32_t>> lists(8);
    for (uint32_t x = 0; x < 8; x++)
        for (uint32_t t0 = 0; t0 < L; t0 += LM_MODDOWN_TGROUP)
            for (uint32_t pw = x; pw < 2 * B; pw += 8)
                for (uint32_t t = t0; t < std::min<uint32_t>(t0 + LM_MODDOWN_TGROUP, L); t++) lists[x].push_back(pw | (t << 16));
    return interleave_work_lists(ctx, lists, (size_t)2 * B * L, "ModDown", tb->d_work_down, cache_key, out);
}

template <int LOGN>
static uint32_t intt_pack_slots(lumen_ctx *ctx) {
    static const uint32_t v = [&] {
        hipDeviceProp_t prop;
        int per_cu = 0;
        if (hipGetDeviceProperties(&prop, ctx->device) != hipSuccess) return 256u;
        (void)hipFuncSetAttribute(reinterpret_cast<const void *>(&k_intt_pack<LOGN>),
                                  hipFuncAttributeMaxDynamicSharedMemorySize, (int)LM_CU_LDS_BYTES);
        constexpr lm_geom g = lm_geom_lds(LOGN);
        if (hipOccupancyMaxActiveBlocksPerMultiprocessor(&per_cu, k_intt_pack<LOGN>, g.threads, g.lds) != hipSuccess || per_cu < 1) {
            per_cu = (int)std::max<size_t>(1, std::min<size_t>(LM_CU_LDS_BYTES / g.lds, 2048 / g.threads));
        }
        (void)hipGetLastError();
        if (ctx->tune.debug)
            fprintf(stderr, "[lumenos_hip] k_intt_pack<%d>: %d workgroup(s) per CU, %d CUs\n", LOGN, per_cu,
                    prop.multiProcessorCount);
        return (uint32_t)prop.multiProcessorCount * (uint32_t)per_cu;
    }();
    return v;
}
static uint32_t ks_fused_digits(lumen_ctx *ctx, uint32_t B, uint32_t L) {
    if (lm_is_split(ctx->logN)) return 0;
    const long forced = ctx->tune.ks_fused_digits;
    const uint32_t pairs = L / 2;
    if (forced >= 0) return std::min<uint32_t>((uint32_t)forced, pairs);
    uint32_t slots = 0;
    if (lm_for_logn(ctx, ctx->logN, [&](auto n) { return slots = intt_pack_slots<n>(ctx), 0; })) return 0;
    for (uint32_t nf = pairs; nf >= 1; nf--)
        if (((uint64_t)B * nf) % slots == 0) return nf;
    return 0;
}

static int launch_ks_mac(lumen_ctx *ctx, const u64 *ext, const u64 *acc, const u64 *key, u64 *u, uint32_t B, KsTables *tb) {
    const uint32_t L = tb->nl, K = ctx->K, pshift = ctx->L - L, key_beta = (ctx->L + K - 1) / K;
    const dim3 grid(((ctx->N / LM_MAC_VEC + 255) / 256) * (L + K) * ((B + LM_MAC_COLS - 1) / LM_MAC_COLS));
    hipLaunchKernelGGL(k_ks_mac, grid, dim3(256), 0, ctx->stream, ext, acc, key, u, B, L, K, tb->beta, pshift, key_beta, ctx->logN,
                       ctx->mods);
    LM_HIP(ctx, hipGetLastError());
    return 0;
}

template <bool ACCUMULATE>
static int launch_moddown(lumen_ctx *ctx, const u64 *in, u64 *out, uint32_t B, const lm_galois_key &gk, KsTables *tb,
                          const KsScratch &s) {
    const uint32_t L = tb->nl, K = ctx->K;
    const uint32_t *work_down = nullptr;
    if (int rc = moddown_work_list(ctx, tb, B, &work_down)) return rc;
    lm_prof_scope ps(ctx, ACCUMULATE ? "ks_moddown_ntt" : "ks_rotdown_ntt", (uint64_t)B * 2 * L);
    return lm_for_any_logn(ctx, ctx->logN, [&](auto n) {
        constexpr int LN = decltype(n)::value;
        return lm_launch(ctx, ACCUMULATE ? k_moddown_ntt<LN> : k_rotdown_ntt<LN>, lm_geom_fwd(LN), lm_fwd_grid<LN>(B * 2 * L), s.u, in, out, tb->d_bxp.get(), tb->d_pinv.get(),
                         gk.d_index.get(), gk.d_inv_index.get(), work_down, B, L, K, ctx->mods, ctx->sh->tw_fwd.get());
    });
}

}

int rotate_decompose(lumen_ctx *ctx, const u64 *acc, uint32_t B, KsTables *tb, const KsScratch &s) {
    const uint32_t N = ctx->N, L = tb->nl, K = ctx->K, beta = tb->beta;
    const uint32_t pshift = ctx->L - L;
    const uint32_t nf = K == 2 ? ks_fused_digits(ctx, B, L) : 0;
    if (nf) {
        const uint32_t grid = B * nf + B * (L - 2 * nf);
        lm_prof_scope ps(ctx, "ks_intt_c1", (uint64_t)B * L);
        if (int rc = lm_for_logn(ctx, ctx->logN, [&](auto n) {
                return lm_launch(ctx, k_intt_pack<n>, lm_geom_lds(n), grid, acc, s.coef, B, L, nf, ctx->mods, tb->yscale,
                                 ctx->sh->tw_inv.get());
            }))
            return rc;
    } else {
        if (int rc = lm_launch_ntt_strided(ctx, acc + (size_t)L * N, (size_t)2 * L * N, s.coef, (size_t)L * N, B,
                                           lm_map_q(L), true, "ks_intt_c1", &tb->yscale))
            return rc;
    }
    if (K == 2 && nf < beta) {
        lm_prof_scope ps(ctx, "ks_pack_v", (uint64_t)B);
        if (int rc = lm_launch_pack_v(ctx, s.coef + (size_t)2 * nf * N, (size_t)L * N, B, beta - nf, K, 2 * nf, L - 2 * nf)) return rc;
    }
    {
        const uint64_t nb = (uint64_t)B * tb->pairs.size();
        const uint32_t *work = nullptr;
        if (int rc = modup_work_list(ctx, tb, B, &work)) return rc;
        lm_prof_scope ps(ctx, "ks_modup_ntt", nb);
        if (int rc = lm_for_any_logn(ctx, ctx->logN, [&](auto n) {
                return lm_launch(ctx, k_modup_ntt<n>, lm_geom_fwd(n), lm_fwd_grid<n>((uint32_t)nb), s.coef, acc, s.ext, tb->d_bx.get(), B, L, K, beta,
                                 pshift, work, ctx->mods, ctx->sh->tw_fwd.get());
            }))
            return rc;
    }
    return 0;
}

int rotate_product(lumen_ctx *ctx, const u64 *acc, uint32_t B, const lm_galois_key &gk, KsTables *tb, const KsScratch &s) {
    if (int rc = rotate_mac(ctx, acc, B, gk, tb, s)) return rc;
    return rotate_p_to_coef(ctx, s.u, B, tb);
}

int rotate_mac(lumen_ctx *ctx, const u64 *acc, uint32_t B, const lm_galois_key &gk, KsTables *tb, const KsScratch &s) {
    lm_prof_scope ps(ctx, "ks_mac", (uint64_t)B);
    return launch_ks_mac(ctx, s.ext, acc, gk.d_key.get(), s.u, B, tb);
}

int rotate_p_to_coef(lumen_ctx *ctx, u64 *u, uint32_t B, KsTables *tb) {
    const uint32_t N = ctx->N, L = tb->nl, K = ctx->K;
    u64 *up = u + ks_u_at(0, L, B, L, K) * N;
    const size_t pstride = (size_t)K * N;
    if (int rc = lm_launch_ntt_strided(ctx, up, pstride, up, pstride, B * 2, lm_map_p(ctx), true, "ks_intt_p",
                                       &tb->yscale))
        return rc;
    if (K == 2) {
        lm_prof_scope ps(ctx, "ks_pack_v", (uint64_t)B);
        if (int rc = lm_launch_pack_v(ctx, up, pstride, B * 2, 1u, K, ctx->L, K)) return rc;
    }
    return 0;
}

int rotate_accumulate(lumen_ctx *ctx, const u64 *acc, u64 *acc_out, uint32_t B, const lm_galois_key &gk,
                      KsTables *tb, const KsScratch &s) {
    if (int rc = rotate_decompose(ctx, acc, B, tb, s)) return rc;
    return rotate_add(ctx, acc, acc_out, B, gk, tb, s);
}

int rotate_add(lumen_ctx *ctx, const u64 *acc, u64 *acc_out, uint32_t B, const lm_galois_key &gk, KsTables *tb, const KsScratch &s) {
    if (int rc = rotate_product(ctx, acc, B, gk, tb, s)) return rc;
    return launch_moddown<true>(ctx, acc, acc_out, B, gk, tb, s);
}

int rotate_store(lumen_ctx *ctx, const u64 *in, u64 *out, uint32_t B, const lm_galois_key &gk, KsTables *tb, const KsScratch &s) {
    return launch_moddown<false>(ctx, in, out, B, gk, tb, s);
}

int rotate_close(lumen_ctx *ctx, const u64 *acc, u64 *coef_out, uint32_t B, const lm_galois_key &gk, uint64_t gal_el,
                 KsTables *tb, const KsScratch &s) {
    if (int rc = rotate_product(ctx, acc, B, gk, tb, s)) return rc;
    const uint32_t *work_down = nullptr;
    if (int rc = moddown_work_list(ctx, tb, B, &work_down)) return rc;
    return ks_close_launch(ctx, acc, coef_out, B, gk, gal_el, tb, s, work_down);
}

extern "C" int lumen_ks_mac_probe(lumen_ctx *ctx, uint32_t batch, const void *ext, const void *acc, const void *key,
                                  void *u, uint32_t reps, float *ms_per_launch) {
    LM_CHECK(nullptr, ctx && ms_per_launch, "lumen_ks_mac_probe: NULL argument");
    LM_ENTER(ctx);
    KsTables *tb = nullptr;
    if (int rc = get_tables(ctx, &tb)) return rc;
    const uint32_t N = ctx->N, L = ctx->L, B = batch ? batch : ks_batch(ctx);
    LM_CHECK(ctx, B <= 65535 && reps >= 1 && reps <= 100000, "lumen_ks_mac_probe: batch %u / reps %u out of range", B, reps);
    KsScratch s;
    if (int rc = get_scratch(ctx, B, tb, &s)) return rc;
    if (!acc) acc = lm_scratch(ctx, "ks_acc", (size_t)B * 2 * L * N * 8);
    if (!acc) return 1;
    if (!key) {
        LM_SHARED_LOCK(ctx);
        LM_CHECK(ctx, !ctx->gkeys.empty(), "lumen_ks_mac_probe: no Galois key loaded");
        key = ctx->gkeys.begin()->second.d_key.get();
    }
    const u64 *pe = ext ? (const u64 *)ext : s.ext;
    u64 *pu = u ? (u64 *)u : s.u;
    auto launch = [&] { return launch_ks_mac(ctx, pe, (const u64 *)acc, (const u64 *)key, pu, B, tb); };
    for (int i = 0; i < 3; i++)
        if (int rc = launch()) return rc;
    LM_HIP(ctx, hipEventRecord(ctx->tm0, ctx->stream));
    for (uint32_t i = 0; i < reps; i++)
        if (int rc = launch()) return rc;
    LM_HIP(ctx, hipEventRecord(ctx->tm1, ctx->stream));
    LM_HIP(ctx, hipEventSynchronize(ctx->tm1));
    float ms = 0;
    LM_HIP(ctx, hipEventElapsedTime(&ms, ctx->tm0, ctx->tm1));
    *ms_per_launch = ms / (float)reps;
    return 0;
}
```

lumenos_amd/csrc/lm_ks_close.hip:

```cpp
#include "lm_ks_host.h"

#ifndef LM_KS_CLOSE_PF
#define LM_KS_CLOSE_PF 4
#endif

template <int LOGN>
__global__ LM_GEOM_BOUNDS(lm_geom_lds(LOGN)) void k_ks_close(const u64 *__restrict__ u, const u64 *__restrict__ acc_in,
                                                              u64 *__restrict__ out, const bx_t *__restrict__ bxp,
                                                              const tw_t *__restrict__ pinv,
                                                              const uint32_t *__restrict__ index,
                                                              const uint32_t *__restrict__ inv_index, uint32_t ginv,
                                                              const uint32_t *__restrict__ work, uint32_t B, uint32_t L,
                                                              uint32_t K, lm_mods mods, lm_ninv_t ninv,
                                                              const tw_t *__restrict__ tw_all) {
    extern __shared__ __attribute__((aligned(16))) u64 sm[];
    constexpr uint32_t N = 1u << LOGN;
    const uint32_t tid = threadIdx.x;
    const uint32_t wk = work[blockIdx.x];
    const uint32_t pw = wk & 0xFFFF;
    const uint32_t t = wk >> 16;
    const uint32_t w = pw & 1;
    const bx_t c = bxp[t];
    const lm_qc qc = lm_make_qc(mods.m[t]);
    const u64 *up0 = u + ks_u_at(pw, L, B, L, K) * N;
    const u64 *up1 = c.ns == 2 ? up0 + N : up0;
    const u64 *uq = u + ks_u_at(pw, t, B, L, K) * N;
    const u64 *ain = acc_in + ((size_t)pw * L + t) * N;
    u64 *o = out + ((size_t)pw * L + t) * N;
    constexpr uint32_t NW = lm_nthreads(LOGN) / 64, BLK = N / NW, IT = BLK / 128, CH = IT < 4 ? IT : 4;
    static_assert(IT >= 1 && IT % CH == 0, "a wave stages its block as pairs of words, 128 per instruction");
    {
        const uint32_t wave = tid >> 6, lane = tid & 63;
        const uint32_t sb = NW > 1 ? (uint32_t)__builtin_amdgcn_readfirstlane((int)(index[wave * BLK] / BLK)) : 0u;
#pragma unroll
        for (uint32_t k0 = 0; k0 < IT; k0 += CH) {
            uint2 p[CH];
            ulonglong2 x[CH], c0[CH];
#pragma unroll
            for (uint32_t k = 0; k < CH; k++) {
                const uint32_t s = sb * BLK + 2 * lane + (k0 + k) * 128;
                p[k] = *reinterpret_cast<const uint2 *>(inv_index + s);
                x[k] = *reinterpret_cast<const ulonglong2 *>(uq + s);
                if (w == 0) c0[k] = *reinterpret_cast<const ulonglong2 *>(ain + s);
            }
#pragma unroll
            for (uint32_t k = 0; k < CH; k++) {
                sm[LM_PAD(wave * BLK + (p[k].x & (BLK - 1)))] = w == 0 ? x[k].x + c0[k].x : x[k].x;
                sm[LM_PAD(wave * BLK + (p[k].y & (BLK - 1)))] = w == 0 ? x[k].y + c0[k].y : x[k].y;
            }
        }
        lm_wave_sync();
    }
    auto ld = [&](uint32_t j0, u64 *v, int count) {
        lm_load_run(ain, j0, v, count);
#pragma unroll
        for (int k = 0; k < 8; k++)
            if (k < count) {
                const u64 x = sm[LM_PAD(j0 + k)];
                v[k] = w == 0 ? lm_csub(v[k] + x, 2 * qc.q) : v[k] + x;
            }
    };
    constexpr int R_LAST = lm_pass_r(LOGN, 0), LOG_T0 = LOGN - R_LAST, CNT = 1 << R_LAST;
    constexpr int PF = LM_KS_CLOSE_PF < CNT ? LM_KS_CLOSE_PF : CNT;
    tw_t npi = pinv[t];
    npi.w = qc.q - npi.w, npi.wp = ~npi.wp;
    struct close_t {
        u64 *o;
        const u64 *up0, *up1;
        const bx_t &c;
        const lm_qc &qc;
        tw_t ni, npi;
        uint32_t ginv;
        u64 hi[PF], lo[PF];
        __device__ __forceinline__ uint32_t src(uint32_t i) const { return (ginv * i) & (2 * N - 1); }
        __device__ __forceinline__ void fetch(uint32_t i, u64 &h, u64 &l) const {
            const uint32_t s = src(i) & (N - 1);
            h = up0[s], l = up1[s];
        }
        __device__ __forceinline__ void pre(uint32_t w0) {
#pragma unroll
            for (int k = 0; k < PF; k++) fetch(w0 + ((uint32_t)k << LOG_T0), hi[k], lo[k]);
        }
        __device__ __forceinline__ void operator()(uint32_t i, u64 v, int k) {
            const u64 h = hi[k % PF], l = lo[k % PF];
            if (k + PF < CNT) fetch(i + ((uint32_t)PF << LOG_T0), hi[k % PF], lo[k % PF]);
            const u64 m = lm_shoup3<true>(bx_apply(c, h, l, qc), npi.w, npi.wp, qc.nq);
            const u64 r = lm_shoup3<true>(v, ni.w, ni.wp, qc.nq);
            u64 y = r + (src(i) >= N ? qc.q3 - m : m);
            y = lm_csub(lm_csub(y, 4 * qc.q), 2 * qc.q);
            o[i] = lm_csub(y, qc.q);
        }
    } st{o, up0, up1, c, qc, ninv.t[t], npi, ginv, {}, {}};
    lm_ntt_inverse<LOGN>(sm, tw_all + (size_t)t * N, qc, tid, ld, st);
}

static uint32_t inv_mod_2n(uint64_t g, uint32_t N) {
    uint64_t x = g;
    for (int i = 0; i < 5; i++) x *= 2 - g * x;
    return (uint32_t)(x & (2ull * N - 1));
}

int ks_close_launch(lumen_ctx *ctx, const u64 *acc, u64 *out, uint32_t B, const lm_galois_key &gk, uint64_t gal_el,
                    KsTables *tb, const KsScratch &s, const uint32_t *work_down) {
    const uint32_t L = tb->nl, K = ctx->K;
    const uint32_t ginv = inv_mod_2n(gal_el, ctx->N);
    lm_prof_scope ps(ctx, "rescale_intt", (uint64_t)B * 2 * L);
    return lm_for_logn(ctx, ctx->logN, [&](auto n) {
        return lm_launch(ctx, k_ks_close<n>, lm_geom_lds(n), B * 2 * L, s.u, acc, out, tb->d_bxp.get(), tb->d_pinv.get(),
                         gk.d_index.get(), gk.d_inv_index.get(), ginv, work_down, B, L, K, ctx->mods, lm_ninv_of(ctx), ctx->sh->tw_inv.get());
    });
}
```

lumenos_amd/csrc/lm_ks_dev.h:

```cpp
#pragma once
#include "lm_ntt_dev.h"

struct bx_t {
    tw_t b57;
    u64 c_t;
    uint32_t ns;
    uint32_t own;
};
#define LM_W_SPLIT 57

__device__ __forceinline__ u64 bx_apply(const bx_t &c, u64 a, u64 b, const lm_qc &qc) {
    if (c.ns == 1) return lm_shoup3<true>(a, 1ull, qc.qinv64, qc.nq);
    return lm_shoup3<true>(a, c.b57.w, c.b57.wp, qc.nq, b + c.c_t);
}

__host__ __device__ __forceinline__ size_t ks_ext_at(uint32_t b, uint32_t d, uint32_t t, uint32_t B, uint32_t beta) {
    return ((size_t)t * B + b) * beta + d;
}
__host__ __device__ __forceinline__ size_t ks_u_at(uint32_t pw, uint32_t t, uint32_t B, uint32_t L, uint32_t K) {
    return t < L ? (size_t)t * 2 * B + pw : (size_t)L * 2 * B + (size_t)pw * K + (t - L);
}
__host__ __device__ __forceinline__ size_t ks_key_at(uint32_t d, uint32_t w, uint32_t t, uint32_t beta) {
    return ((size_t)t * beta + d) * 2 + w;
}

__host__ __device__ __forceinline__ uint32_t ks_mod_at(uint32_t t, uint32_t nl, uint32_t pshift) {
    return t < nl ? t : t + pshift;
}

__device__ __forceinline__ void mul128(u64 a, u64 b, u64 &lo, u64 &hi) {
    const u32 a0 = (u32)a, a1 = (u32)(a >> 32), b0 = (u32)b, b1 = (u32)(b >> 32);
    const u64 p0 = (u64)a0 * b0;
    const u64 p1 = lm_keep((u64)a0 * b1 + (p0 >> 32));
    const u64 p2 = lm_keep((u64)a1 * b0 + (u32)p1);
    hi = (u64)a1 * b1 + (p1 >> 32) + (p2 >> 32);
    lo = (p2 << 32) | (u32)p0;
}

struct lm_ks_view {
    const bx_t *d_bxp;
    const tw_t *d_pinv;
    const lm_ninv_t *yscale;
};
int lm_ks_tables_view(lumen_ctx *ctx, lm_ks_view *out);
int lm_launch_pack_v(lumen_ctx *ctx, u64 *y, size_t poly_stride, uint32_t npoly, uint32_t ngroups,
                     uint32_t group_limbs, uint32_t first_mod, uint32_t nlimbs_total);
```

lumenos_amd/csrc/lm_ks_host.h:

```cpp
#pragma once
#include "lm_ks_dev.h"

struct KsTables {
    lm_dev<bx_t> d_bx;
    lm_dev<bx_t> d_bxp;
    lm_dev<tw_t> d_pinv;
    uint32_t nl = 0;
    uint32_t beta = 0;
    lm_ninv_t yscale;
    std::vector<uint16_t> pairs;
    std::map<uint32_t, lm_dev<uint32_t>> d_work;
    std::map<uint32_t, lm_dev<uint32_t>> d_work_down;
};
int get_tables(lumen_ctx *ctx, KsTables **out);
int get_tables_at(lumen_ctx *ctx, uint32_t nl, KsTables **out);

struct KsScratch {
    u64 *coef, *ext, *u, *acc2;
};

int rotate_decompose(lumen_ctx *ctx, const u64 *acc, uint32_t B, KsTables *tb, const KsScratch &s);
int rotate_product(lumen_ctx *ctx, const u64 *acc, uint32_t B, const lm_galois_key &gk, KsTables *tb, const KsScratch &s);
int rotate_mac(lumen_ctx *ctx, const u64 *acc, uint32_t B, const lm_galois_key &gk, KsTables *tb, const KsScratch &s);
int rotate_p_to_coef(lumen_ctx *ctx, u64 *u, uint32_t B, KsTables *tb);
int rotate_add(lumen_ctx *ctx, const u64 *acc, u64 *acc_out, uint32_t B, const lm_galois_key &gk, KsTables *tb, const KsScratch &s);
int rotate_accumulate(lumen_ctx *ctx, const u64 *acc, u64 *acc_out, uint32_t B, const lm_galois_key &gk,
                      KsTables *tb, const KsScratch &s);
int rotate_store(lumen_ctx *ctx, const u64 *in, u64 *out, uint32_t B, const lm_galois_key &gk, KsTables *tb, const KsScratch &s);
int rotate_close(lumen_ctx *ctx, const u64 *acc, u64 *coef_out, uint32_t B, const lm_galois_key &gk, uint64_t gal_el,
                 KsTables *tb, const KsScratch &s);
int ks_close_launch(lumen_ctx *ctx, const u64 *acc, u64 *out, uint32_t B, const lm_galois_key &gk, uint64_t gal_el,
                    KsTables *tb, const KsScratch &s, const uint32_t *work_down);
int get_scratch(lumen_ctx *ctx, uint32_t B, KsTables *tb, KsScratch *s, int lane = 0, u64 **group_acc = nullptr,
                size_t group_acc_bytes = 0);

int upload_ptT(lumen_ctx *ctx, const uint64_t *pt, uint32_t nl, u64 **out);
int launch_mul_plain(lumen_ctx *ctx, const u64 *ct, u64 *out, const u64 *ptT, size_t words, uint32_t nl,
                     uint32_t ncts);

std::shared_ptr<lm_galois_key> lm_relin_key(lumen_ctx *ctx);
int ks_find_key(lumen_ctx *ctx, uint64_t gal_el, const lm_galois_key **gk);
int check_level_of_chain(lumen_ctx *ctx, const lumen_set *in, const char *what);
uint32_t ks_batch(const lumen_ctx *ctx);
uint32_t ks_lanes(const lumen_ctx *ctx);
struct LaneGuard {
    lumen_ctx *ctx;
    hipStream_t saved;
    LaneGuard(lumen_ctx *c, int lane) : ctx(c), saved(c->stream) {
        if (lane) ctx->stream = ctx->stream2;
    }
    ~LaneGuard() { ctx->stream = saved; }
};

struct KsRun {
    KsTables *top = nullptr, *tb = nullptr;
    uint32_t Bmax = 0, group = 0, lanes = 1;
    bool grouped = false;
    size_t group_bytes = 0;
    KsScratch s[2] = {};
    u64 *acc = nullptr;
};
int ks_run_open(lumen_ctx *ctx, uint32_t count, uint32_t nl, uint32_t max_lanes, bool group_acc, KsRun *run);
int ks_run_scratch(lumen_ctx *ctx, KsRun *run);
template <class Batch, class Group>
int ks_run(lumen_ctx *ctx, const KsRun &run, uint32_t count, size_t ctw, Batch &&batch, Group &&end_of_group) {
    for (uint32_t g0 = 0; g0 < count; g0 += run.group) {
        const uint32_t gn = std::min(run.group, count - g0);
        if (run.lanes > 1) {
            LM_HIP(ctx, hipEventRecord(ctx->ev_fork, ctx->stream));
            LM_HIP(ctx, hipStreamWaitEvent(ctx->stream2, ctx->ev_fork, 0));
        }
        uint32_t lane = 0;
        for (uint32_t first = 0; first < gn; first += run.Bmax, lane = (lane + 1) % run.lanes) {
            const uint32_t B = std::min(run.Bmax, gn - first);
            LaneGuard guard(ctx, (int)lane);
            if (int rc = batch(g0, first, B, run.s[lane], run.acc ? run.acc + (size_t)first * ctw : nullptr)) return rc;
        }
        if (run.lanes > 1) {
            LM_HIP(ctx, hipEventRecord(ctx->ev_join, ctx->stream2));
            LM_HIP(ctx, hipStreamWaitEvent(ctx->stream, ctx->ev_join, 0));
        }
        if (int rc = end_of_group(g0, gn)) return rc;
    }
    return 0;
}
template <class Batch>
int ks_run(lumen_ctx *ctx, const KsRun &run, uint32_t count, size_t ctw, Batch &&batch) {
    return ks_run(ctx, run, count, ctw, batch, [](uint32_t, uint32_t) { return 0; });
}
```

Before: 1.688 s.

## Fold c0 key-switch lifts into 192-bit accumulator across InnerSum rotations

Adds a c0-fold path for InnerSum rotation chains. Instead of running ModDown on both ciphertext halves each rotation, the c0 lift contributions are accumulated in a 192-bit per-coefficient sum carried across rotations, and only the c1 half goes through ModDown. The gadget-product kernel also directly computes the rotated c0 add into the output accumulator. This aims to cut roughly half the ModDown NTT work per rotation, at the cost of extra 3-word scratch traffic and a more complex correctness argument about overflow bounds.

```diff
diff --git a/lumenos_amd/csrc/lm_common.h b/lumenos_amd/csrc/lm_common.h
--- a/lumenos_amd/csrc/lm_common.h
+++ b/lumenos_amd/csrc/lm_common.h
@@ -66,6 +66,7 @@
     uint32_t ks_lanes = 0;
     int32_t ks_fused_digits = -1;
     uint32_t ks_close_fused = 1;
+    uint32_t ks_c0_fold = 1;
     uint32_t debug = 0;
     uint32_t modup_tgroup = 3, moddown_tgroup = 1;
     uint32_t ks_placement = 6;
diff --git a/lumenos_amd/csrc/lm_ctx.hip b/lumenos_amd/csrc/lm_ctx.hip
--- a/lumenos_amd/csrc/lm_ctx.hip
+++ b/lumenos_amd/csrc/lm_ctx.hip
@@ -180,6 +180,9 @@
     } else if (n == "LUMEN_KS_CLOSE_FUSED") {
         if (!in(0, 1)) return 2;
         t.ks_close_fused = (uint32_t)v;
+    } else if (n == "LUMEN_KS_C0_FOLD") {
+        if (!in(0, 1)) return 2;
+        t.ks_c0_fold = (uint32_t)v;
     } else if (n == "LUMEN_DEBUG") {
         t.debug = v != 0;
     } else if (n == "LUMEN_MODUP_TGROUP") {
@@ -200,7 +203,7 @@
     return 0;
 }
 static void tuning_from_env(lm_tuning &t) {
-    for (const char *n : {"LUMEN_KS_BATCH", "LUMEN_KS_LANES", "LUMEN_KS_FUSED_DIGITS", "LUMEN_KS_CLOSE_FUSED", "LUMEN_DEBUG",
+    for (const char *n : {"LUMEN_KS_BATCH", "LUMEN_KS_LANES", "LUMEN_KS_FUSED_DIGITS", "LUMEN_KS_CLOSE_FUSED", "LUMEN_KS_C0_FOLD", "LUMEN_DEBUG",
                           "LUMEN_MODUP_TGROUP", "LUMEN_MODDOWN_TGROUP", "LUMEN_KS_PLACEMENT", "LUMEN_BATCH_CHUNKS"}) {
         const char *e = getenv(n);
         if (e && *e && tuning_set(t, n, atol(e)))
diff --git a/lumenos_amd/csrc/lm_innersum.hip b/lumenos_amd/csrc/lm_innersum.hip
--- a/lumenos_amd/csrc/lm_innersum.hip
+++ b/lumenos_amd/csrc/lm_innersum.hip
@@ -72,6 +72,7 @@
 struct SumPlan {
     struct Step {
         const lm_galois_key *dbl = nullptr, *term = nullptr;
+        uint64_t dbl_el = 0;
     } it[32];
     uint32_t cnt = 0;
     uint64_t last_el = 0;
@@ -85,7 +86,7 @@
             if (int rc = ks_find_key(ctx, term, &st.term)) return rc;
             p->lazy = true;
         }
-        p->last_el = dbl;
+        p->last_el = st.dbl_el = dbl;
         return ks_find_key(ctx, dbl, &st.dbl);
     });
 }
@@ -143,13 +144,23 @@
 }
 
 int inner_sum_batch(lumen_ctx *ctx, u64 *acc, uint32_t B, const SumPlan &plan, KsTables *tb, const KsScratch &s, u64 *lazy,
-                    u64 *close_out) {
+                    u64 *close_out, u64 *fold_s = nullptr) {
     LM_CHECK(ctx, !close_out || (plan.cnt && !plan.lazy), "InnerSum has no rotation to close");
+    LM_CHECK(ctx, !fold_s || (close_out && ks_fold_serves(ctx, tb, plan.cnt)),
+             "the c0 fold cannot hold the lifts of %u rotations of %u bits in 192", plan.cnt, tb->lift_bits);
     u64 *cur = acc, *other = s.acc2;
     bool first = true;
     for (uint32_t r = 0; r < plan.cnt; r++) {
         const SumPlan::Step &st = plan.it[r];
         if (int rc = rotate_decompose(ctx, cur, B, tb, s)) return rc;
+        if (fold_s) {
+            const u64 *s_in = r ? fold_s + ((r - 1) & 1) * ks_fold_words(ctx, B) : nullptr;
+            u64 *s_out = fold_s + (r & 1) * ks_fold_words(ctx, B);
+            if (r + 1 == plan.cnt) return rotate_close_fold(ctx, cur, close_out, B, *st.dbl, st.dbl_el, tb, s, s_in, s_out);
+            if (int rc = rotate_add_fold(ctx, cur, other, B, *st.dbl, st.dbl_el, tb, s, s_in, s_out)) return rc;
+            std::swap(cur, other);
+            continue;
+        }
         if (st.term) {
             if (int rc = rotate_mac(ctx, cur, B, *st.term, tb, s)) return rc;
             if (int rc = lazy_gather(ctx, s.u, cur, lazy, st.term->d_index.get(), first, B, tb)) return rc;
@@ -239,10 +250,18 @@
         if (rc && rc != 2) return rc;
         close = rc == 0;
     }
+    u64 *fold_s[2] = {nullptr, nullptr};
+    if (close && ctx->tune.ks_c0_fold && ks_fold_serves(ctx, run.tb, plan.cnt)) {
+        const size_t bytes = 2 * ks_fold_words(ctx, run.Bmax) * 8;
+        fold_s[0] = (u64 *)lm_scratch(ctx, "ks_fold_s", bytes);
+        fold_s[1] = run.lanes > 1 ? (u64 *)lm_scratch(ctx, "ks_fold_s_b", bytes) : fold_s[0];
+        if (!fold_s[0] || !fold_s[1]) return 1;
+    }
     auto batch_fn = [&](uint32_t g0, uint32_t first, uint32_t B, const KsScratch &s, u64 *a) {
         if (int rc = launch_mul_plain(ctx, matrix->d + (size_t)(g0 + first) * ctw, a, ptT, (size_t)B * ctw, L, B))
             return rc;
-        return inner_sum_batch(ctx, a, B, plan, run.tb, s, lazy[&s == &run.s[1]], close ? work + (size_t)first * ctw : nullptr);
+        const int lane = &s == &run.s[1];
+        return inner_sum_batch(ctx, a, B, plan, run.tb, s, lazy[lane], close ? work + (size_t)first * ctw : nullptr, fold_s[lane]);
     };
     auto end_of_group = [&](uint32_t g0, uint32_t gn) {
         if (close)
diff --git a/lumenos_amd/csrc/lm_keyswitch.hip b/lumenos_amd/csrc/lm_keyswitch.hip
--- a/lumenos_amd/csrc/lm_keyswitch.hip
+++ b/lumenos_amd/csrc/lm_keyswitch.hip
@@ -241,86 +241,12 @@
 #endif
 }
 
-__global__ __launch_bounds__(256) void k_ks_mac(const u64 *__restrict__ ext, const u64 *__restrict__ acc,
-                                                const u64 *__restrict__ key, u64 *__restrict__ u, uint32_t B,
-                                                uint32_t L, uint32_t K, uint32_t beta, uint32_t pshift,
-                                                uint32_t key_beta, uint32_t logN, lm_mods mods) {
-    typedef mac_vec<LM_MAC_VEC> vec;
-    const uint32_t N = 1u << logN, LK = L + K;
-    const uint32_t G = (B + LM_MAC_COLS - 1) / LM_MAC_COLS, per_limb = N / (256 * LM_MAC_VEC) ? N / (256 * LM_MAC_VEC) : 1;
-    const uint32_t slices = per_limb * LK;
-    uint32_t slice, z;
-    if (slices % 8 == 0) {
-        const uint32_t xcd = blockIdx.x & 7, j = blockIdx.x >> 3;
-        z = j % G;
-        slice = (j / G) * 8 + xcd;
-    } else {
-        z = blockIdx.x % G;
-        slice = blockIdx.x / G;
-    }
-    const uint32_t i = ((slice % per_limb) * 256 + threadIdx.x) * LM_MAC_VEC;
-    const uint32_t t = LK - 1 - slice / per_limb;
-    const uint32_t mt = ks_mod_at(t, L, pshift);
-    const uint32_t b0 = z * LM_MAC_COLS;
-    if (i >= N) return;
-    const mod_t md = mods.m[mt];
-    const uint32_t own = t < L ? t / K : 0xFFFFFFFFu;
-    mac_acc a0[LM_MAC_COLS][LM_MAC_VEC], a1[LM_MAC_COLS][LM_MAC_VEC];
-#pragma unroll
-    for (int c = 0; c < LM_MAC_COLS; c++)
-#pragma unroll
-        for (int e = 0; e < LM_MAC_VEC; e++) a0[c][e].clear(), a1[c][e].clear();
-    struct digit_t {
-        vec k0, k1, x[LM_MAC_COLS];
-    };
-    auto fetch = [&](uint32_t d) {
-        digit_t g;
-        g.k0 = vec::load(key + ks_key_at(d, 0, mt, key_beta) * N + i);
-        g.k1 = vec::load(key + ks_key_at(d, 1, mt, key_beta) * N + i);
-#pragma unroll
-        for (int c = 0; c < LM_MAC_COLS; c++) {
-            const uint32_t bc = b0 + c < B ? b0 + c : B - 1;
-            g.x[c] = d == own ? vec::load(acc + ((size_t)(bc * 2 + 1) * L + t) * N + i)
-                              : vec::load_once(ext + ks_ext_at(bc, d, t, B, beta) * N + i);
-        }
-        return g;
-    };
-    constexpr int PF = LM_MAC_PREFETCH;
-    digit_t q[PF + 1];
-#pragma unroll
-    for (int j = 0; j < PF; j++)
-        if ((uint32_t)j < beta) q[j] = fetch(j);
-    for (uint32_t d0 = 0; d0 < beta; d0 += PF + 1) {
-#pragma unroll
-        for (int j = 0; j <= PF; j++) {
-            const uint32_t d = d0 + j;
-            if (d < beta) {
-                if (d + PF < beta) q[(j + PF) % (PF + 1)] = fetch(d + PF);
-#pragma unroll
-                for (int c = 0; c < LM_MAC_COLS; c++)
-#pragma unroll
-                    for (int e = 0; e < LM_MAC_VEC; e++) mac2(a0[c][e], a1[c][e], q[j].x[c].v[e], q[j].k0.v[e], q[j].k1.v[e]);
-            }
-        }
-    }
-#pragma unroll
-    for (int c = 0; c < LM_MAC_COLS; c++) {
-        if (b0 + c < B) {
-            u64 *o = u + ks_u_at((b0 + c) * 2, t, B, L, K) * N + i, *o1 = u + ks_u_at((b0 + c) * 2 + 1, t, B, L, K) * N + i;
-            vec r0, r1;
-#pragma unroll
-            for (int e = 0; e < LM_MAC_VEC; e++) {
-                u64 lo, hi;
-                a0[c][e].value(lo, hi);
-                r0.v[e] = lm_mont_reduce_wide(lo, hi, md.q, md.qneg, md.qinv64, beta);
-                a1[c][e].value(lo, hi);
-                r1.v[e] = lm_mont_reduce_wide(lo, hi, md.q, md.qneg, md.qinv64, beta);
-            }
-            r0.store(o);
-            r1.store(o1);
-        }
-    }
-}
+#define LM_KS_MAC_FOLD 0
+#include "lm_ks_mac_kernel.h"
+#undef LM_KS_MAC_FOLD
+#define LM_KS_MAC_FOLD 1
+#include "lm_ks_mac_kernel.h"
+#undef LM_KS_MAC_FOLD
 
 template <int LOGN, bool ACCUMULATE>
 __device__ __forceinline__ void moddown_body(const u64 *__restrict__ u, const u64 *__restrict__ acc_in,
@@ -535,13 +461,27 @@
         const uint64_t q = ctx->mod[t];
         pinv[t] = h_tw(h_invmod(h_p_mod(ctx, q), q), q);
     }
+    {
+        unsigned __int128 M = 1;
+        for (uint32_t a = 0; a < K; a++) M *= ctx->mod[ctx->L + a];
+        const unsigned __int128 bound = K == 2 ? 2 * M : M;
+        tb.m2_lo = K == 2 ? (u64)(2 * M) : 0, tb.m2_hi = K == 2 ? (u64)((2 * M) >> 64) : 0;
+        for (tb.lift_bits = 0; tb.lift_bits < 128 && (bound >> tb.lift_bits); tb.lift_bits++) {}
+    }
+    std::vector<sfold_t> sfold(L);
+    for (uint32_t t = 0; t < L; t++) {
+        const uint64_t q = ctx->mod[t];
+        const uint64_t r63 = (1ull << 63) % q, r64 = h_mulmod(r63, 2 % q, q), r128 = h_mulmod(r64, r64, q);
+        sfold[t].r64 = h_tw(r64, q), sfold[t].r128 = h_tw(r128, q);
+        sfold[t].off = q - h_mulmod(r63, r128, q), sfold[t].pad = 0;
+    }
     std::vector<uint16_t> pairs;
     for (uint32_t t = 0; t < LK; t++)
         for (uint32_t d = 0; d < tb.beta; d++)
             if (!bx[(size_t)d * LK + t].own) pairs.push_back((uint16_t)(d | (t << 8)));
     tb.pairs = pairs;
     if (tb.d_bx.upload(ctx, bx, "the key switch's extension constants") || tb.d_bxp.upload(ctx, bxp, "the key switch's lift constants") ||
-        tb.d_pinv.upload(ctx, pinv, "the key switch's P^-1 table"))
+        tb.d_pinv.upload(ctx, pinv, "the key switch's P^-1 table") || tb.d_sfold.upload(ctx, sfold, "the c0 fold's reduction constants"))
         return 1;
     ctx->ext[name] = sp;
     *out = sp.get();
@@ -612,11 +552,11 @@
     return interleave_work_lists(ctx, lists, (size_t)B * tb->pairs.size(), "extension", tb->d_work, cache_key, out);
 }
 
-static int moddown_work_list(lumen_ctx *ctx, KsTables *tb, uint32_t B, const uint32_t **out) {
+static int moddown_work_list(lumen_ctx *ctx, KsTables *tb, uint32_t B, const uint32_t **out, bool c1_only = false) {
     const uint32_t LM_MODDOWN_TGROUP = ctx->tune.moddown_tgroup;
     LM_SHARED_LOCK(ctx);
     LM_CHECK(ctx, B >= 1 && 2 * (uint64_t)B <= 65535, "key-switch batch of %u columns does not fit the packed work list", B);
-    const uint32_t cache_key = B | (LM_MODDOWN_TGROUP << 17);
+    const uint32_t cache_key = B | (LM_MODDOWN_TGROUP << 17) | (c1_only ? 1u << 31 : 0u);
     auto it = tb->d_work_down.find(cache_key);
     if (it != tb->d_work_down.end()) {
         *out = it->second.get();
@@ -626,9 +566,9 @@
     std::vector<std::vector<uint32_t>> lists(8);
     for (uint32_t x = 0; x < 8; x++)
         for (uint32_t t0 = 0; t0 < L; t0 += LM_MODDOWN_TGROUP)
-            for (uint32_t pw = x; pw < 2 * B; pw += 8)
+            for (uint32_t pw = c1_only ? 2 * x + 1 : x; pw < 2 * B; pw += c1_only ? 16 : 8)
                 for (uint32_t t = t0; t < std::min<uint32_t>(t0 + LM_MODDOWN_TGROUP, L); t++) lists[x].push_back(pw | (t << 16));
-    return interleave_work_lists(ctx, lists, (size_t)2 * B * L, "ModDown", tb->d_work_down, cache_key, out);
+    return interleave_work_lists(ctx, lists, (size_t)(c1_only ? 1 : 2) * B * L, "ModDown", tb->d_work_down, cache_key, out);
 }
 
 template <int LOGN>
@@ -671,17 +611,28 @@
     LM_HIP(ctx, hipGetLastError());
     return 0;
 }
+static int launch_ks_mac_fold(lumen_ctx *ctx, const u64 *ext, const u64 *acc, const lm_galois_key &gk, u64 *u, u64 *acc_out, uint32_t B,
+                              KsTables *tb) {
+    const uint32_t L = tb->nl, K = ctx->K, pshift = ctx->L - L, key_beta = (ctx->L + K - 1) / K;
+    LM_CHECK(ctx, ctx->N >= 256 && LM_MAC_VEC == 1, "the folded gadget product works on blocks of 256 coefficients");
+    const dim3 grid((ctx->N / 256) * (L + K) * ((B + LM_MAC_COLS - 1) / LM_MAC_COLS));
+    hipLaunchKernelGGL(k_ks_mac_fold, grid, dim3(256), 0, ctx->stream, ext, acc, gk.d_key.get(), u, B, L, K, tb->beta, pshift, key_beta,
+                       ctx->logN, ctx->mods, acc_out, gk.d_index.get(), gk.d_inv_index.get());
+    LM_HIP(ctx, hipGetLastError());
+    return 0;
+}
 
 template <bool ACCUMULATE>
 static int launch_moddown(lumen_ctx *ctx, const u64 *in, u64 *out, uint32_t B, const lm_galois_key &gk, KsTables *tb,
-                          const KsScratch &s) {
+                          const KsScratch &s, bool c1_only = false) {
     const uint32_t L = tb->nl, K = ctx->K;
     const uint32_t *work_down = nullptr;
-    if (int rc = moddown_work_list(ctx, tb, B, &work_down)) return rc;
-    lm_prof_scope ps(ctx, ACCUMULATE ? "ks_moddown_ntt" : "ks_rotdown_ntt", (uint64_t)B * 2 * L);
+    if (int rc = moddown_work_list(ctx, tb, B, &work_down, c1_only)) return rc;
+    const uint32_t items = (c1_only ? 1 : 2) * B * L;
+    lm_prof_scope ps(ctx, ACCUMULATE ? "ks_moddown_ntt" : "ks_rotdown_ntt", (uint64_t)items);
     return lm_for_any_logn(ctx, ctx->logN, [&](auto n) {
         constexpr int LN = decltype(n)::value;
-        return lm_launch(ctx, ACCUMULATE ? k_moddown_ntt<LN> : k_rotdown_ntt<LN>, lm_geom_fwd(LN), lm_fwd_grid<LN>(B * 2 * L), s.u, in, out, tb->d_bxp.get(), tb->d_pinv.get(),
+        return lm_launch(ctx, ACCUMULATE ? k_moddown_ntt<LN> : k_rotdown_ntt<LN>, lm_geom_fwd(LN), lm_fwd_grid<LN>(items), s.u, in, out, tb->d_bxp.get(), tb->d_pinv.get(),
                          gk.d_index.get(), gk.d_inv_index.get(), work_down, B, L, K, ctx->mods, ctx->sh->tw_fwd.get());
     });
 }
@@ -770,6 +721,34 @@
     return ks_close_launch(ctx, acc, coef_out, B, gk, gal_el, tb, s, work_down);
 }
 
+#ifndef LM_KS_FOLD_MIN_ROTATIONS
+#define LM_KS_FOLD_MIN_ROTATIONS 3
+#endif
+bool ks_fold_serves(const lumen_ctx *ctx, const KsTables *tb, uint32_t rotations) {
+    return ctx->N >= 256 && !lm_is_split(ctx->logN) && ctx->K >= 1 && ctx->K <= 2 && rotations >= LM_KS_FOLD_MIN_ROTATIONS &&
+           rotations + tb->lift_bits <= 191;
+}
+
+int rotate_add_fold(lumen_ctx *ctx, const u64 *acc, u64 *acc_out, uint32_t B, const lm_galois_key &gk, uint64_t gal_el, KsTables *tb,
+                    const KsScratch &s, const u64 *s_in, u64 *s_out) {
+    {
+        lm_prof_scope ps(ctx, "ks_mac", (uint64_t)B);
+        if (int rc = launch_ks_mac_fold(ctx, s.ext, acc, gk, s.u, acc_out, B, tb)) return rc;
+    }
+    if (int rc = rotate_p_to_coef(ctx, s.u, B, tb)) return rc;
+    if (int rc = lift_fold_launch(ctx, s.u, s_in, s_out, B, gal_el, tb)) return rc;
+    return launch_moddown<true>(ctx, acc, acc_out, B, gk, tb, s, true);
+}
+
+int rotate_close_fold(lumen_ctx *ctx, const u64 *acc, u64 *coef_out, uint32_t B, const lm_galois_key &gk, uint64_t gal_el,
+                      KsTables *tb, const KsScratch &s, const u64 *s_in, u64 *s_out) {
+    if (int rc = rotate_product(ctx, acc, B, gk, tb, s)) return rc;
+    if (int rc = lift_fold_launch(ctx, s.u, s_in, s_out, B, gal_el, tb)) return rc;
+    const uint32_t *work_down = nullptr;
+    if (int rc = moddown_work_list(ctx, tb, B, &work_down)) return rc;
+    return ks_close_launch(ctx, acc, coef_out, B, gk, gal_el, tb, s, work_down, s_out);
+}
+
 extern "C" int lumen_ks_mac_probe(lumen_ctx *ctx, uint32_t batch, const void *ext, const void *acc, const void *key,
                                   void *u, uint32_t reps, float *ms_per_launch) {
     LM_CHECK(nullptr, ctx && ms_per_launch, "lumen_ks_mac_probe: NULL argument");
diff --git a/lumenos_amd/csrc/lm_ks_close.hip b/lumenos_amd/csrc/lm_ks_close.hip
--- a/lumenos_amd/csrc/lm_ks_close.hip
+++ b/lumenos_amd/csrc/lm_ks_close.hip
@@ -4,7 +4,7 @@
 #define LM_KS_CLOSE_PF 4
 #endif
 
-template <int LOGN>
+template <int LOGN, bool FOLD>
 __global__ LM_GEOM_BOUNDS(lm_geom_lds(LOGN)) void k_ks_close(const u64 *__restrict__ u, const u64 *__restrict__ acc_in,
                                                               u64 *__restrict__ out, const bx_t *__restrict__ bxp,
                                                               const tw_t *__restrict__ pinv,
@@ -12,7 +12,9 @@
                                                               const uint32_t *__restrict__ inv_index, uint32_t ginv,
                                                               const uint32_t *__restrict__ work, uint32_t B, uint32_t L,
                                                               uint32_t K, lm_mods mods, lm_ninv_t ninv,
-                                                              const tw_t *__restrict__ tw_all) {
+                                                              const tw_t *__restrict__ tw_all,
+                                                              const u64 *__restrict__ fold_s,
+                                                              const sfold_t *__restrict__ sfc) {
     extern __shared__ __attribute__((aligned(16))) u64 sm[];
     constexpr uint32_t N = 1u << LOGN;
     const uint32_t tid = threadIdx.x;
@@ -71,26 +73,37 @@
         const lm_qc &qc;
         tw_t ni, npi;
         uint32_t ginv;
-        u64 hi[PF], lo[PF];
+        const u64 *sp;
+        sfold_t sf;
+        u64 hi[PF], lo[PF], top[FOLD ? PF : 1];
         __device__ __forceinline__ uint32_t src(uint32_t i) const { return (ginv * i) & (2 * N - 1); }
-        __device__ __forceinline__ void fetch(uint32_t i, u64 &h, u64 &l) const {
+        __device__ __forceinline__ void fetch(uint32_t i, u64 &h, u64 &l, u64 &x) const {
+            if (FOLD && sp) {
+                h = sp[i], l = sp[N + i], x = sp[2 * N + i];
+                return;
+            }
             const uint32_t s = src(i) & (N - 1);
             h = up0[s], l = up1[s];
         }
         __device__ __forceinline__ void pre(uint32_t w0) {
 #pragma unroll
-            for (int k = 0; k < PF; k++) fetch(w0 + ((uint32_t)k << LOG_T0), hi[k], lo[k]);
+            for (int k = 0; k < PF; k++) fetch(w0 + ((uint32_t)k << LOG_T0), hi[k], lo[k], top[FOLD ? k : 0]);
         }
         __device__ __forceinline__ void operator()(uint32_t i, u64 v, int k) {
-            const u64 h = hi[k % PF], l = lo[k % PF];
-            if (k + PF < CNT) fetch(i + ((uint32_t)PF << LOG_T0), hi[k % PF], lo[k % PF]);
-            const u64 m = lm_shoup3<true>(bx_apply(c, h, l, qc), npi.w, npi.wp, qc.nq);
+            const u64 h = hi[k % PF], l = lo[k % PF], x = top[FOLD ? k % PF : 0];
+            if (k + PF < CNT) fetch(i + ((uint32_t)PF << LOG_T0), hi[k % PF], lo[k % PF], top[FOLD ? k % PF : 0]);
             const u64 r = lm_shoup3<true>(v, ni.w, ni.wp, qc.nq);
-            u64 y = r + (src(i) >= N ? qc.q3 - m : m);
+            u64 y;
+            if (FOLD && sp) {
+                y = r + lm_shoup3<true>(lm_s192_mod(sf, h, l, x, qc), npi.w, npi.wp, qc.nq);
+            } else {
+                const u64 m = lm_shoup3<true>(bx_apply(c, h, l, qc), npi.w, npi.wp, qc.nq);
+                y = r + (src(i) >= N ? qc.q3 - m : m);
+            }
             y = lm_csub(lm_csub(y, 4 * qc.q), 2 * qc.q);
             o[i] = lm_csub(y, qc.q);
         }
-    } st{o, up0, up1, c, qc, ninv.t[t], npi, ginv, {}, {}};
+    } st{o, up0, up1, c, qc, ninv.t[t], npi, ginv, FOLD && w == 0 ? fold_s + (size_t)(pw >> 1) * 3 * N : nullptr, FOLD ? sfc[t] : sfold_t{}, {}, {}, {}};
     lm_ntt_inverse<LOGN>(sm, tw_all + (size_t)t * N, qc, tid, ld, st);
 }
 
@@ -101,12 +114,58 @@
 }
 
 int ks_close_launch(lumen_ctx *ctx, const u64 *acc, u64 *out, uint32_t B, const lm_galois_key &gk, uint64_t gal_el,
-                    KsTables *tb, const KsScratch &s, const uint32_t *work_down) {
+                    KsTables *tb, const KsScratch &s, const uint32_t *work_down, const u64 *fold_s) {
     const uint32_t L = tb->nl, K = ctx->K;
     const uint32_t ginv = inv_mod_2n(gal_el, ctx->N);
     lm_prof_scope ps(ctx, "rescale_intt", (uint64_t)B * 2 * L);
     return lm_for_logn(ctx, ctx->logN, [&](auto n) {
-        return lm_launch(ctx, k_ks_close<n>, lm_geom_lds(n), B * 2 * L, s.u, acc, out, tb->d_bxp.get(), tb->d_pinv.get(),
-                         gk.d_index.get(), gk.d_inv_index.get(), ginv, work_down, B, L, K, ctx->mods, lm_ninv_of(ctx), ctx->sh->tw_inv.get());
+        constexpr int LN = decltype(n)::value;
+        auto go = [&](auto kernel) {
+            return lm_launch(ctx, kernel, lm_geom_lds(LN), B * 2 * L, s.u, acc, out, tb->d_bxp.get(), tb->d_pinv.get(), gk.d_index.get(),
+                             gk.d_inv_index.get(), ginv, work_down, B, L, K, ctx->mods, lm_ninv_of(ctx), ctx->sh->tw_inv.get(), fold_s,
+                             tb->d_sfold.get());
+        };
+        return fold_s ? go(k_ks_close<LN, true>) : go(k_ks_close<LN, false>);
     });
 }
+
+__global__ __launch_bounds__(256) void k_lift_fold(const u64 *__restrict__ up, const u64 *__restrict__ s_in, u64 *__restrict__ s_out,
+                                                   uint32_t ginv, uint32_t B, uint32_t K, uint32_t logN, u64 m2_lo, u64 m2_hi) {
+    const uint32_t N = 1u << logN, C = N >> 8;
+    uint32_t b, chunk;
+    if (B % 8 == 0) {
+        const uint32_t xcd = blockIdx.x & 7, j = blockIdx.x >> 3;
+        b = (j / C) * 8 + xcd, chunk = j % C;
+    } else {
+        b = blockIdx.x / C, chunk = blockIdx.x % C;
+    }
+    {
+        const uint32_t i = chunk * 256 + threadIdx.x;
+        const uint32_t e = (ginv * i) & (2 * N - 1), s = e & (N - 1);
+        const u64 *w = up + ((size_t)2 * b * K << logN);
+        lm_s192 d;
+        if (K == 2) {
+            const u64 hi = w[s], lo = w[N + s];
+            d = lm_s192_add(lm_s192{lo | (hi << LM_W_SPLIT), hi >> (64 - LM_W_SPLIT), 0}, lm_s192_neg(lm_s192{m2_lo, m2_hi, 0}));
+        } else {
+            d = lm_s192{w[s], 0, 0};
+        }
+        const u64 *pi = s_in ? s_in + (size_t)b * 3 * N : nullptr;
+        u64 *po = s_out + (size_t)b * 3 * N;
+        if (s_in) d = lm_s192_add(d, lm_s192{pi[s], pi[N + s], pi[2 * N + s]});
+        if (e >= N) d = lm_s192_neg(d);
+        if (s_in) d = lm_s192_add(d, lm_s192{pi[i], pi[N + i], pi[2 * N + i]});
+        po[i] = d.a, po[N + i] = d.b, po[2 * N + i] = d.c;
+    }
+}
+
+int lift_fold_launch(lumen_ctx *ctx, const u64 *u, const u64 *s_in, u64 *s_out, uint32_t B, uint64_t gal_el, KsTables *tb) {
+    const uint32_t L = tb->nl, K = ctx->K;
+    LM_CHECK(ctx, s_out && s_out != s_in, "the folded lifts need a block of their own");
+    LM_CHECK(ctx, ctx->N >= 256, "the lift fold works on blocks of 256 coefficients");
+    lm_prof_scope ps(ctx, "ks_lift_fold", (uint64_t)B);
+    hipLaunchKernelGGL(k_lift_fold, dim3(B * (ctx->N / 256)), dim3(256), 0, ctx->stream,
+                       u + ks_u_at(0, L, B, L, K) * ctx->N, s_in, s_out, inv_mod_2n(gal_el, ctx->N), B, K, ctx->logN, tb->m2_lo, tb->m2_hi);
+    LM_HIP(ctx, hipGetLastError());
+    return 0;
+}
diff --git a/lumenos_amd/csrc/lm_ks_dev.h b/lumenos_amd/csrc/lm_ks_dev.h
--- a/lumenos_amd/csrc/lm_ks_dev.h
+++ b/lumenos_amd/csrc/lm_ks_dev.h
@@ -12,6 +12,34 @@
 __device__ __forceinline__ u64 bx_apply(const bx_t &c, u64 a, u64 b, const lm_qc &qc) {
     if (c.ns == 1) return lm_shoup3<true>(a, 1ull, qc.qinv64, qc.nq);
     return lm_shoup3<true>(a, c.b57.w, c.b57.wp, qc.nq, b + c.c_t);
+}
+
+struct lm_s192 {
+    u64 a, b, c;
+};
+__host__ __device__ __forceinline__ lm_s192 lm_s192_add(const lm_s192 &x, const lm_s192 &y) {
+    lm_s192 r;
+    r.a = x.a + y.a;
+    const u64 c0 = r.a < x.a ? 1u : 0u;
+    r.b = x.b + y.b;
+    u64 c1 = r.b < x.b ? 1u : 0u;
+    r.b += c0;
+    c1 += r.b < c0 ? 1u : 0u;
+    r.c = x.c + y.c + c1;
+    return r;
+}
+__host__ __device__ __forceinline__ lm_s192 lm_s192_neg(const lm_s192 &x) {
+    return lm_s192_add(lm_s192{~x.a, ~x.b, ~x.c}, lm_s192{1, 0, 0});
+}
+struct sfold_t {
+    tw_t r64, r128;
+    u64 off, pad;
+};
+__device__ __forceinline__ u64 lm_s192_mod(const sfold_t &f, u64 s0, u64 s1, u64 s2, const lm_qc &qc) {
+    const u64 r0 = lm_shoup3<true>(s0, 1ull, qc.qinv64, qc.nq);
+    const u64 r1 = lm_shoup3<true>(s1, f.r64.w, f.r64.wp, qc.nq);
+    const u64 r2 = lm_shoup3<true>(s2 ^ (1ull << 63), f.r128.w, f.r128.wp, qc.nq);
+    return r0 + r1 + r2 + f.off;
 }
 
 __host__ __device__ __forceinline__ size_t ks_ext_at(uint32_t b, uint32_t d, uint32_t t, uint32_t B, uint32_t beta) {
diff --git a/lumenos_amd/csrc/lm_ks_host.h b/lumenos_amd/csrc/lm_ks_host.h
--- a/lumenos_amd/csrc/lm_ks_host.h
+++ b/lumenos_amd/csrc/lm_ks_host.h
@@ -5,6 +5,9 @@
     lm_dev<bx_t> d_bx;
     lm_dev<bx_t> d_bxp;
     lm_dev<tw_t> d_pinv;
+    lm_dev<sfold_t> d_sfold;
+    u64 m2_lo = 0, m2_hi = 0;
+    uint32_t lift_bits = 0;
     uint32_t nl = 0;
     uint32_t beta = 0;
     lm_ninv_t yscale;
@@ -30,7 +33,15 @@
 int rotate_close(lumen_ctx *ctx, const u64 *acc, u64 *coef_out, uint32_t B, const lm_galois_key &gk, uint64_t gal_el,
                  KsTables *tb, const KsScratch &s);
 int ks_close_launch(lumen_ctx *ctx, const u64 *acc, u64 *out, uint32_t B, const lm_galois_key &gk, uint64_t gal_el,
-                    KsTables *tb, const KsScratch &s, const uint32_t *work_down);
+                    KsTables *tb, const KsScratch &s, const uint32_t *work_down, const u64 *fold_s = nullptr);
+
+bool ks_fold_serves(const lumen_ctx *ctx, const KsTables *tb, uint32_t rotations);
+inline size_t ks_fold_words(const lumen_ctx *ctx, uint32_t B) { return (size_t)B * 3 * ctx->N; }
+int rotate_add_fold(lumen_ctx *ctx, const u64 *acc, u64 *acc_out, uint32_t B, const lm_galois_key &gk, uint64_t gal_el, KsTables *tb,
+                    const KsScratch &s, const u64 *s_in, u64 *s_out);
+int rotate_close_fold(lumen_ctx *ctx, const u64 *acc, u64 *coef_out, uint32_t B, const lm_galois_key &gk, uint64_t gal_el,
+                      KsTables *tb, const KsScratch &s, const u64 *s_in, u64 *s_out);
+int lift_fold_launch(lumen_ctx *ctx, const u64 *u, const u64 *s_in, u64 *s_out, uint32_t B, uint64_t gal_el, KsTables *tb);
 int get_scratch(lumen_ctx *ctx, uint32_t B, KsTables *tb, KsScratch *s, int lane = 0, u64 **group_acc = nullptr,
                 size_t group_acc_bytes = 0);
 
diff --git a/lumenos_amd/csrc/lm_ks_mac_kernel.h b/lumenos_amd/csrc/lm_ks_mac_kernel.h
--- /dev/null
+++ b/lumenos_amd/csrc/lm_ks_mac_kernel.h
@@ -0,0 +1,121 @@
+#if LM_KS_MAC_FOLD
+__global__ __launch_bounds__(256) void k_ks_mac_fold(const u64 *__restrict__ ext, const u64 *__restrict__ acc,
+                                                     const u64 *__restrict__ key, u64 *__restrict__ u, uint32_t B,
+                                                     uint32_t L, uint32_t K, uint32_t beta, uint32_t pshift,
+                                                     uint32_t key_beta, uint32_t logN, lm_mods mods,
+                                                     u64 *__restrict__ acc_out, const uint32_t *__restrict__ index,
+                                                     const uint32_t *__restrict__ inv_index) {
+#else
+__global__ __launch_bounds__(256) void k_ks_mac(const u64 *__restrict__ ext, const u64 *__restrict__ acc,
+                                                const u64 *__restrict__ key, u64 *__restrict__ u, uint32_t B,
+                                                uint32_t L, uint32_t K, uint32_t beta, uint32_t pshift,
+                                                uint32_t key_beta, uint32_t logN, lm_mods mods) {
+#endif
+    typedef mac_vec<LM_MAC_VEC> vec;
+    const uint32_t N = 1u << logN, LK = L + K;
+    const uint32_t G = (B + LM_MAC_COLS - 1) / LM_MAC_COLS, per_limb = N / (256 * LM_MAC_VEC) ? N / (256 * LM_MAC_VEC) : 1;
+    const uint32_t slices = per_limb * LK;
+    uint32_t slice, z;
+    if (slices % 8 == 0) {
+        const uint32_t xcd = blockIdx.x & 7, j = blockIdx.x >> 3;
+        z = j % G;
+        slice = (j / G) * 8 + xcd;
+    } else {
+        z = blockIdx.x % G;
+        slice = blockIdx.x / G;
+    }
+    const uint32_t i = ((slice % per_limb) * 256 + threadIdx.x) * LM_MAC_VEC;
+    const uint32_t t = LK - 1 - slice / per_limb;
+    const uint32_t mt = ks_mod_at(t, L, pshift);
+    const uint32_t b0 = z * LM_MAC_COLS;
+    if (i >= N) return;
+    const mod_t md = mods.m[mt];
+    const uint32_t own = t < L ? t / K : 0xFFFFFFFFu;
+    mac_acc a0[LM_MAC_COLS][LM_MAC_VEC], a1[LM_MAC_COLS][LM_MAC_VEC];
+#pragma unroll
+    for (int c = 0; c < LM_MAC_COLS; c++)
+#pragma unroll
+        for (int e = 0; e < LM_MAC_VEC; e++) a0[c][e].clear(), a1[c][e].clear();
+    struct digit_t {
+        vec k0, k1, x[LM_MAC_COLS];
+    };
+    auto fetch = [&](uint32_t d) {
+        digit_t g;
+        g.k0 = vec::load(key + ks_key_at(d, 0, mt, key_beta) * N + i);
+        g.k1 = vec::load(key + ks_key_at(d, 1, mt, key_beta) * N + i);
+#pragma unroll
+        for (int c = 0; c < LM_MAC_COLS; c++) {
+            const uint32_t bc = b0 + c < B ? b0 + c : B - 1;
+            g.x[c] = d == own ? vec::load(acc + ((size_t)(bc * 2 + 1) * L + t) * N + i)
+                              : vec::load_once(ext + ks_ext_at(bc, d, t, B, beta) * N + i);
+        }
+        return g;
+    };
+    constexpr int PF = LM_MAC_PREFETCH;
+    digit_t q[PF + 1];
+#pragma unroll
+    for (int j = 0; j < PF; j++)
+        if ((uint32_t)j < beta) q[j] = fetch(j);
+    for (uint32_t d0 = 0; d0 < beta; d0 += PF + 1) {
+#pragma unroll
+        for (int j = 0; j <= PF; j++) {
+            const uint32_t d = d0 + j;
+            if (d < beta) {
+                if (d + PF < beta) q[(j + PF) % (PF + 1)] = fetch(d + PF);
+#pragma unroll
+                for (int c = 0; c < LM_MAC_COLS; c++)
+#pragma unroll
+                    for (int e = 0; e < LM_MAC_VEC; e++) mac2(a0[c][e], a1[c][e], q[j].x[c].v[e], q[j].k0.v[e], q[j].k1.v[e]);
+            }
+        }
+    }
+#if LM_KS_MAC_FOLD
+    u64 u0[LM_MAC_COLS];
+#endif
+#pragma unroll
+    for (int c = 0; c < LM_MAC_COLS; c++) {
+        if (b0 + c < B) {
+            u64 *o = u + ks_u_at((b0 + c) * 2, t, B, L, K) * N + i, *o1 = u + ks_u_at((b0 + c) * 2 + 1, t, B, L, K) * N + i;
+            vec r0, r1;
+#pragma unroll
+            for (int e = 0; e < LM_MAC_VEC; e++) {
+                u64 lo, hi;
+                a0[c][e].value(lo, hi);
+                r0.v[e] = lm_mont_reduce_wide(lo, hi, md.q, md.qneg, md.qinv64, beta);
+                a1[c][e].value(lo, hi);
+                r1.v[e] = lm_mont_reduce_wide(lo, hi, md.q, md.qneg, md.qinv64, beta);
+            }
+#if LM_KS_MAC_FOLD
+            if (t >= L) r0.store(o);
+            u0[c] = r0.v[0];
+#else
+            r0.store(o);
+#endif
+            r1.store(o1);
+        }
+    }
+#if LM_KS_MAC_FOLD
+    {
+        static_assert(LM_MAC_VEC == 1, "the fold parks one coefficient per thread");
+        __shared__ u64 park[LM_MAC_COLS][256];
+        if (t < L) {
+            const uint32_t i0 = i - threadIdx.x;
+            const uint32_t j = (inv_index[i0] & ~255u) + threadIdx.x;
+            const uint32_t src = index[j] & 255u;
+            u64 aj[LM_MAC_COLS];
+#pragma unroll
+            for (int c = 0; c < LM_MAC_COLS; c++)
+                if (b0 + c < B) {
+                    const u64 *a = acc + ((size_t)(b0 + c) * 2 * L + t) * N;
+                    park[c][threadIdx.x] = a[i] + u0[c];
+                    aj[c] = a[j];
+                }
+            __syncthreads();
+#pragma unroll
+            for (int c = 0; c < LM_MAC_COLS; c++)
+                if (b0 + c < B)
+                    acc_out[((size_t)(b0 + c) * 2 * L + t) * N + j] = lm_csub(lm_csub(aj[c] + park[c][src], 4 * md.q), 2 * md.q);
+        }
+    }
+#endif
+}
```

Result: faster. 1.621 s, median of 6 (-4.0%).
